# intuitive-robots/mdt_policy

Hardware: AMD Instinct MI355X
Metric: action-chunks/sec (10-step denoise, horizon=10) (higher is better)
Workload: dtype f32

## Files before the change

### include/mdt_hip_ops.h

```cpp
#ifndef MDT_HIP_OPS_H
#define MDT_HIP_OPS_H

#include <stdint.h>
#include "mdt_hip.h"

#ifdef __cplusplus
extern "C" {
#endif

enum { MDT_ACT_NONE = 0, MDT_ACT_GELU = 1, MDT_ACT_MISH = 2, MDT_ACT_SILU = 3,
       MDT_ACT_SWIGLU = 4  };
enum { MDT_HEAD_DENOISED = 0, MDT_HEAD_DDIM = 1, MDT_HEAD_RAW = 2,
       MDT_HEAD_PLAN = 3  };

int64_t mdt_op_packed_numel(int64_t N, int64_t K);

mdt_status mdt_op_pack_weight(const float *w, int64_t n_rows, int64_t K, float *packed, int64_t n_off,
                              int64_t N_total, void *stream);
mdt_status mdt_op_pack_weight_glu(const float *w, int64_t H2, int64_t K, float *packed, void *stream);

typedef struct {
    const float *A;
    int64_t lda;
    const float *Wp;
    const float *bias;
    float *out;
    int64_t ldo;
    int32_t M, N, K;
    int32_t ln;
    const float *ln_w, *ln_b;
    const float *mod;
    int64_t mod_stride;
    int32_t shift_off, scale_off;
    int32_t rows_per_sample;
    int32_t act;
    int32_t residual;
    int32_t gate_off;
    int32_t gin, gout, goff;
    const float *rowvec;
    int32_t batch;
    int64_t bs_a, bs_w, bs_out;
    const float *aux;
    int32_t aux_mode;
    int32_t a_parts;
    int64_t a_part_stride;
    float *a_merged;
    const void *Wp_split;
} mdt_gemm_args;

mdt_status mdt_op_gemm(const mdt_gemm_args *args, void *stream);

mdt_status mdt_op_mlp(const mdt_gemm_args *fc, const mdt_gemm_args *proj, float *parts, int64_t part_stride,
                      int32_t *n_parts, void *stream);
mdt_status mdt_op_pack_weight_split(const float *w, int64_t n_rows, int64_t K, void *image, void *stream);
mdt_status mdt_op_pack_weight_split_rows(const float *w, int64_t n_rows, int64_t K, void *image, int64_t n_off, void *stream);
mdt_status mdt_op_mlp_split(const mdt_gemm_args *fc, const mdt_gemm_args *proj, const void *fc_split, const void *proj_split,
                            float *parts, int64_t part_stride, int32_t *n_parts, void *stream);
void mdt_op_set_mlp_split(int32_t on);
void mdt_op_set_mlp_fuse_min(int32_t rows);
void mdt_op_set_side_jobs(int32_t on);
int64_t mdt_op_side_jobs_paired(void);
void mdt_op_trace_mlp(int32_t enable);
int32_t mdt_op_trace_mlp_read(float *us, int32_t cap);
int32_t mdt_op_trace_mlp_read_empty(float *us, int32_t cap);
mdt_status mdt_op_clock_stamp(uint64_t *out16, void *stream);
void mdt_op_set_ws_split(int32_t on);

void mdt_op_set_mlp_skew(int32_t v);

void mdt_op_set_gemm_geometry(int32_t geometry);

typedef struct {
    const float *q; int64_t ldq;
    const float *k; const float *v;
    int64_t ldkv;
    float *out; int64_t ldo;
    int32_t B, H, hd, Tq, Tk;
    int32_t causal;
    int32_t rope;
} mdt_attn_args;

mdt_status mdt_op_attention(const mdt_attn_args *args, void *stream);

mdt_status mdt_op_attn_proj(const mdt_gemm_args *proj, const float *qkv, int64_t ldq, int32_t hd, int32_t T, int32_t causal,
                            void *stream);
void mdt_op_set_attn_wide_min(int32_t rows);

mdt_status mdt_op_layernorm(const float *in, const float *w, const float *b, float *out, int64_t M, int32_t D,
                            void *stream);

typedef struct {
    const float *y;
    const float *ln_w;
    const float *ln_b;
    const float *Wp, *bp;
    const float *x;
    const float *sigma;
    int64_t sigma_stride;
    float *out;
    int32_t M, D, A, rows_per_sample;
    int32_t mode;
    const float *step;
    float sigma_data;
    float *y_next;
    const float *Wa, *ba;
    int32_t no_ln;
    int32_t y_parts;
    int64_t y_part_stride;
} mdt_head_args;

mdt_status mdt_op_head(const mdt_head_args *args, void *stream);

typedef struct {
    const float *kv; int64_t ldkv;
    const float *WqT_p;
    const float *bq;
    const float *Wo_p;
    float *U, *Wf;
    float *c;
    int32_t B, H, hd, D, Te;
} mdt_xfold_args;
mdt_status mdt_op_xattn_fold(const mdt_xfold_args *args, void *stream);

typedef struct {
    float *y;
    const float *ln_w, *ln_b;
    const float *U, *Wf, *c;
    const float *bo;
    int32_t B, H, D, Te, Ta;
    float *y_out;
} mdt_xapply_args;
mdt_status mdt_op_xattn_apply(const mdt_xapply_args *args, void *stream);

mdt_status mdt_op_xattn_gemm(const mdt_xapply_args *x, const mdt_gemm_args *g, void *stream);

mdt_status mdt_op_attn_xattn(const mdt_gemm_args *proj, const float *qkv, int64_t ldq, const mdt_xapply_args *x, int32_t hd,
                             int32_t T, void *stream);

mdt_status mdt_op_action_embed(const float *x, const float *sigma, int64_t sigma_stride, float sigma_data,
                               const float *WaT, const float *ba, float *y, int64_t M, int32_t A, int32_t D,
// ... 7 lines not shown
```

### mdt_policy_amd/_lib.py

```python
from __future__ import annotations

import ctypes as C
import os
import threading

from . import build as _build

c_float_p = C.POINTER(C.c_float)


class MDTHipError(RuntimeError):
    def __init__(self, status: int, message: str):
        super().__init__(f"libmdt_hip status {status}: {message}")
        self.status = status


class MDTConfig(C.Structure):
    _fields_ = [(n, C.c_int32) for n in (
        "arch", "embed_dim", "n_heads", "n_enc_layers", "n_dec_layers", "action_dim", "obs_dim", "goal_dim",
        "n_obs_token", "goal_seq_len", "action_seq_len", "use_mlp_goal", "use_modality_encoder", "use_abs_pos_emb",
        "use_rot_embed", "use_ada_conditioning", "use_noise_encoder", "linear_output", "bias")] + [
        ("sigma_data", C.c_float), ("no_goal_conditioning", C.c_int32), ("proprio_dim", C.c_int32),
        ("use_proprio", C.c_int32)]

# ... 119 lines not shown


class LinearBwdArgs(C.Structure):
    _fields_ = [("X", C.c_void_p), ("ldx", C.c_int64), ("dY", C.c_void_p), ("ldy", C.c_int64), ("Wt", C.c_void_p),
                ("dW", C.c_void_p), ("dbias", C.c_void_p), ("dX", C.c_void_p), ("ldxo", C.c_int64),
                ("accumulate_dw", C.c_int32), ("accumulate_dx", C.c_int32), ("M", C.c_int32), ("N", C.c_int32),
                ("K", C.c_int32), ("scratch", C.c_void_p), ("dx_act_u", C.c_void_p), ("dx_act", C.c_int32)]


class OptTensor(C.Structure):
    _fields_ = [("p", C.c_void_p), ("g", C.c_void_p), ("m", C.c_void_p), ("v", C.c_void_p), ("ema", C.c_void_p),
                ("numel", C.c_int64)]


class ResamplerConfig(C.Structure):
    _fields_ = [(n, C.c_int32) for n in ("dim", "depth", "dim_head", "heads", "num_latents", "num_time_embeds",
                                          "ff_mult", "activation")]


class MapPoolConfig(C.Structure):
    _fields_ = [(n, C.c_int32) for n in ("n_latents", "embed_dim", "output_dim", "n_heads", "mlp_hidden")]


class InfoNCEArgs(C.Structure):
    _fields_ = [("image_features", C.c_void_p), ("lang_features", C.c_void_p), ("logit_scale", C.c_void_p),
                ("batch", C.c_int32), ("dim", C.c_int32), ("mode", C.c_int32), ("loss", C.c_void_p),
                ("d_image", C.c_void_p), ("d_lang", C.c_void_p), ("d_logit_scale", C.c_void_p), ("scratch", C.c_void_p)]


INFONCE_MODE = {"symmetric": 0, "img_to_text": 1, "text_to_img": 2}
ARCH = {"mdtv": 0, "mdt": 1}
MODALITY = {"vis": 0, "lang": 1}
ACT = {"none": 0, "gelu": 1, "mish": 2, "silu": 3, "swiglu": 4}
HEAD = {"denoised": 0, "ddim": 1, "raw": 2}
RAW_OUTPUT, RAW_INPUT, SIGMA_SCALAR = 1, 2, 4

_VP, _I32, _I64, _F = C.c_void_p, C.c_int32, C.c_int64, C.c_float
SYMBOLS = [
    ("mdt_last_error", C.c_char_p, []),
    ("mdt_version", C.c_char_p, []),
    ("mdt_set_allocator", _I32, [_VP, _VP, _VP]),
    ("mdt_allocator_detach", _I32, []),
    ("mdt_create", _I32, [C.POINTER(MDTConfig), C.POINTER(_VP)]),
    ("mdt_destroy", _I32, [_VP]),
    ("mdt_param_count", _I64, [_VP]),
    ("mdt_param_name", C.c_char_p, [_VP, _I64]),
    ("mdt_param_numel", _I64, [_VP, _I64]),
    ("mdt_load_param", _I32, [_VP, C.c_char_p, _VP, _I64, _VP]),
    ("mdt_load_params", _I32, [_VP, _I32, C.POINTER(C.c_char_p), C.POINTER(C.c_void_p), C.POINTER(_I64), _VP]),
    ("mdt_reserve", _I32, [_VP, _I64]),
    ("mdt_ws_generation", _I64, [_VP]),
    ("mdt_encode", _I32, [_VP, _VP, _VP, _VP, _I32, _I32, _VP, _I64, _VP, _VP]),
    ("mdt_denoise_cached", _I32, [_VP, _VP, _VP, _I64, _I32, _VP, _VP]),
    ("mdt_forward", _I32, [_VP, _VP, _VP, _VP, _I32, _VP, _VP, _I64, _VP, _VP, _VP]),
    ("mdt_sample_ddim", _I32, [_VP, _VP, _VP, _VP, _I32, _VP, C.POINTER(C.c_float), _I32, _I64, _VP, _VP, _VP]),
    ("mdt_sample_ddim_dev", _I32, [_VP, _VP, _VP, _VP, _I32, _VP, _VP, _I32, _I64, _VP, _VP, _VP]),
    ("mdt_sample", _I32, [_VP, _VP, _VP, _VP, _I32, _VP, _I32, C.POINTER(SamplerParams), C.POINTER(C.c_float), _I32, _VP, _I32,
                          _I64, _VP, _VP, _VP]),
    ("mdt_sample_dev", _I32, [_VP, _VP, _VP, _VP, _I32, _VP, _I32, C.POINTER(SamplerParams), _VP, _I32, _VP, _I32, _I64, _VP,
                              _VP, _VP]),
    ("mdt_sampler_plan", _I32, [_I32, C.POINTER(SamplerParams), C.POINTER(C.c_float), _I32, C.POINTER(SamplerPlan)]),
    ("mdt_sample_dpm_adaptive", _I32, [_VP, _VP, _VP, _VP, _I32, _VP, C.c_float, C.c_float, C.POINTER(DpmAdaptiveParams), _I64,
                                       _VP, _VP, C.POINTER(DpmAdaptiveInfo), _VP]),
    ("mdt_dpm_control_init", _I32, [C.POINTER(DpmControl)] + [C.c_double] * 6),
    ("mdt_dpm_control_update", _I32, [C.POINTER(DpmControl), C.c_float, C.POINTER(C.c_int32)]),
    ("mdt_dpm_adaptive_plan", _I32, [_I32, C.c_float, C.c_float, C.POINTER(SamplerPlan)]),
    ("mdt_op_trace_mlp", None, [_I32]),
    ("mdt_op_trace_mlp_read", _I32, [_VP, _I32]),
    ("mdt_op_trace_mlp_read_empty", _I32, [_VP, _I32]),
    ("mdt_op_clock_stamp", _I32, [_VP, _VP]),
    ("mdt_op_set_ws_split", None, [_I32]),
    ("mdt_op_set_tn_split", None, [_I32]),
    ("mdt_loss_fwd", _I32, [_VP, _VP, _VP, _VP, _I32, _VP, _VP, _VP, _I64, _VP, _VP, _VP, _VP]),
    ("mdt_flops_per_chunk", C.c_double, [_VP, _I32]),
    ("mdt_fnv1_32", C.c_uint32, [C.c_char_p, C.c_uint64, C.c_uint32]),
    ("mdt_op_packed_numel", _I64, [_I64, _I64]),
    ("mdt_op_pack_weight", _I32, [_VP, _I64, _I64, _VP, _I64, _I64, _VP]),
    ("mdt_op_pack_weight_glu", _I32, [_VP, _I64, _I64, _VP, _VP]),
    ("mdt_op_gemm", _I32, [C.POINTER(GemmArgs), _VP]),
    ("mdt_op_mlp", _I32, [C.POINTER(GemmArgs), C.POINTER(GemmArgs), _VP, _I64, C.POINTER(_I32), _VP]),
    ("mdt_op_pack_weight_split", _I32, [_VP, _I64, _I64, _VP, _VP]),
    ("mdt_op_pack_weight_split_rows", _I32, [_VP, _I64, _I64, _VP, _I64, _VP]),
    ("mdt_op_mlp_split", _I32, [C.POINTER(GemmArgs), C.POINTER(GemmArgs), _VP, _VP, _VP, _I64, C.POINTER(_I32), _VP]),
    ("mdt_op_set_mlp_split", None, [_I32]),
    ("mdt_op_set_gemm_geometry", None, [_I32]),
    ("mdt_op_set_mlp_fuse_min", None, [_I32]),
    ("mdt_op_set_side_jobs", None, [_I32]),
    ("mdt_op_side_jobs_paired", _I64, []),
    ("mdt_op_set_mlp_skew", None, [_I32]),
    ("mdt_op_set_attn_wide_min", None, [_I32]),
    ("mdt_op_attention", _I32, [C.POINTER(AttnArgs), _VP]),
    ("mdt_op_attn_proj", _I32, [C.POINTER(GemmArgs), _VP, _I64, _I32, _I32, _I32, _VP]),
    ("mdt_op_xattn_fold", _I32, [C.POINTER(XFoldArgs), _VP]),
    ("mdt_op_xattn_apply", _I32, [C.POINTER(XApplyArgs), _VP]),
    ("mdt_op_attn_xattn", _I32, [C.POINTER(GemmArgs), _VP, _I64, C.POINTER(XApplyArgs), _I32, _I32, _VP]),
    ("mdt_op_xattn_gemm", _I32, [C.POINTER(XApplyArgs), C.POINTER(GemmArgs), _VP]),
    ("mdt_op_layernorm", _I32, [_VP, _VP, _VP, _VP, _I64, _I32, _VP]),
    ("mdt_op_head", _I32, [C.POINTER(HeadArgs), _VP]),
    ("mdt_op_action_embed", _I32, [_VP, _VP, _I64, _F, _VP, _VP, _VP, _I64, _I32, _I32, _I32, _VP]),
    ("mdt_train_prepare", _I32, [_VP]),
    ("mdt_grad_numel", _I64, [_VP]),
    ("mdt_grad_offset", _I64, [_VP, _I64]),
    ("mdt_train_loss_fwd", _I32, [_VP, _VP, _VP, _VP, _I32, _VP, _VP, _VP, _I64, C.POINTER(Dropout), _VP, _VP, _VP,
                                  C.POINTER(_I32), _VP]),
    ("mdt_train_loss_bwd", _I32, [_VP, _I32, _VP, _VP, _VP, _VP, _VP, _VP, _VP]),
    ("mdt_train_loss_bwd_stages", _I32, [_VP]),
    ("mdt_train_loss_bwd_stage", _I32, [_VP, _I32, _I32, _VP, _VP, _VP, _VP, _VP, _VP, _VP]),
    ("mdt_train_param_stage", _I32, [_VP, _I64]),
    ("mdt_train_encode_fwd", _I32, [_VP, _VP, _VP, _VP, _I32, _I32, _VP, _I64, C.POINTER(Dropout), _VP, C.POINTER(_I32),
                                    _VP]),
    ("mdt_train_encode_bwd", _I32, [_VP, _I32, _VP, _VP, _VP, _VP, _VP, _VP]),
    ("mdt_tape_release", _I32, [_VP, _I32]),
    ("mdt_denoise_vjp", _I32, [_VP, _VP, _VP, _VP, _I32, _VP, _VP, _VP, _I64, _VP, _VP, _VP]),
    ("mdt_op_pack_weight_t", _I32, [_VP, _I64, _I64, _I64, _VP, _I64, _I64, _VP]),
    ("mdt_op_pack_many", _I32, [_I32, C.POINTER(C.c_void_p), C.POINTER(_I32), C.POINTER(_I32), C.POINTER(C.c_void_p),
                                C.POINTER(C.c_void_p), _VP]),
    ("mdt_op_ln_fwd_train", _I32, [C.POINTER(LnTrainArgs), _VP]),
    ("mdt_op_ln_bwd", _I32, [C.POINTER(LnBwdArgs), _VP]),
    ("mdt_op_attn_bwd", _I32, [C.POINTER(AttnBwdArgs), _VP]),
    ("mdt_op_act_fwd", _I32, [_VP, _VP, _I64, _I32, _VP]),
    ("mdt_op_act_bwd", _I32, [_VP, _VP, _VP, _I64, _I32, _VP]),
    ("mdt_op_attn_fwd_train", _I32, [C.POINTER(AttnTrainArgs), _VP]),
    ("mdt_op_merge_fwd", _I32, [C.POINTER(MergeArgs), _VP]),
    ("mdt_op_merge_bwd", _I32, [C.POINTER(MergeArgs), _VP]),
    ("mdt_op_merge_ln_fwd", _I32, [C.POINTER(MergeArgs), C.POINTER(LnTrainArgs), _VP]),
    ("mdt_op_ln_bwd_merge", _I32, [C.POINTER(LnBwdArgs), C.POINTER(MergeArgs), _VP]),
    ("mdt_op_colsum", _I32, [_VP, _I64, _I64, _I64, _VP, _I32, _VP]),
    ("mdt_op_linear_bwd", _I32, [C.POINTER(LinearBwdArgs), _VP]),
    ("mdt_op_linear_bwd_scratch", _I64, [_I64, _I64, _I64]),
    ("mdt_op_linear_bwd_scratch_exact", _I64, [_I64, _I64, _I64]),
    ("mdt_op_multi_adamw", _I32, [C.POINTER(OptTensor), _I32, _F, _F, _F, _F, _F, _I64, _VP]),
    ("mdt_op_multi_ema", _I32, [C.POINTER(OptTensor), _I32, _F, _VP]),
    ("mdt_resampler_create", _I32, [C.POINTER(ResamplerConfig), C.POINTER(_VP)]),
    ("mdt_resampler_destroy", _I32, [_VP]),
    ("mdt_resampler_param_count", _I64, [_VP]),
    ("mdt_resampler_param_name", C.c_char_p, [_VP, _I64]),
    ("mdt_resampler_param_numel", _I64, [_VP, _I64]),
    ("mdt_resampler_load_param", _I32, [_VP, C.c_char_p, _VP, _I64, _VP]),
    ("mdt_resampler_forward", _I32, [_VP, _VP, _VP, _I64, _I32, _I32, _VP, _VP]),
    ("mdt_resampler_train_prepare", _I32, [_VP]),
    ("mdt_resampler_grad_numel", _I64, [_VP]),
    ("mdt_resampler_grad_offset", _I64, [_VP, _I64]),
    ("mdt_resampler_forward_train", _I32, [_VP, _VP, _VP, _I64, _I32, _I32, _VP, C.POINTER(_I32), _VP]),
    ("mdt_resampler_backward", _I32, [_VP, _I32, _VP, _VP, _VP, _VP]),
    ("mdt_resampler_tape_release", _I32, [_VP, _I32]),
    ("mdt_resampler_flops", C.c_double, [_VP, _I32, _I32]),
    ("mdt_map_pool_create", _I32, [C.POINTER(MapPoolConfig), C.POINTER(_VP)]),
    ("mdt_map_pool_destroy", _I32, [_VP]),
    ("mdt_map_pool_param_count", _I64, [_VP]),
    ("mdt_map_pool_param_name", C.c_char_p, [_VP, _I64]),
    ("mdt_map_pool_param_numel", _I64, [_VP, _I64]),
    ("mdt_map_pool_load_param", _I32, [_VP, C.c_char_p, _VP, _I64, _VP]),
    ("mdt_map_pool_forward", _I32, [_VP, _VP, _I64, _I32, _VP, _VP]),
    ("mdt_map_pool_train_prepare", _I32, [_VP]),
    ("mdt_map_pool_grad_numel", _I64, [_VP]),
    ("mdt_map_pool_grad_offset", _I64, [_VP, _I64]),
    ("mdt_map_pool_forward_train", _I32, [_VP, _VP, _I64, _I32, _VP, C.POINTER(_I32), _VP]),
    ("mdt_map_pool_backward", _I32, [_VP, _I32, _VP, _VP, _VP, _VP]),
    ("mdt_map_pool_tape_release", _I32, [_VP, _I32]),
    ("mdt_op_rms_fwd", _I32, [_VP, _VP, _VP, _I64, _I32, _F, _VP]),
    ("mdt_op_rms_bwd_scratch", _I64, [_I64, _I32]),
    ("mdt_op_rms_bwd", _I32, [_VP, _VP, _VP, _VP, _I32, _VP, _I32, _I64, _I32, _F, _VP, _VP]),
    ("mdt_op_rms_bwd_res", _I32, [_VP, _VP, _VP, _VP, _VP, _VP, _I32, _I64, _I32, _F, _VP, _VP]),
    ("mdt_op_scale_residual_fwd", _I32, [_VP, _VP, _VP, _VP, _I64, _I32, _VP]),
    ("mdt_op_scale_residual_bwd_scratch", _I64, [_I64, _I32]),
    ("mdt_op_scale_residual_bwd", _I32, [_VP, _VP, _VP, _VP, _VP, _I64, _I32, _VP, _VP]),
# ... 114 lines not shown
```

### mdt_policy_amd/csrc/mdt_internal.h

```cpp
#pragma once
#include <hip/hip_runtime.h>
#include <stdint.h>
#include <string.h>

#include "mdt_hip.h"
#include "mdt_hip_ops.h"
#include "mdt_resampler.h"
#include "mdt_hip_train.h"
#include "mdt_mae.h"

mdt_status mdt_fail(mdt_status st, const char* fmt, ...);

#define HIP_TRY(expr)                                                                                       \
    do {                                                                                                    \
        hipError_t _e = (expr);                                                                             \
        if (_e != hipSuccess) return mdt_fail(MDT_ERR_HIP, "%s failed: %s", #expr, hipGetErrorString(_e));  \
    } while (0)

#define MDT_TRY(expr)                      \
    do {                                   \
        mdt_status _s = (expr);            \
        if (_s != MDT_OK) return _s;       \
    } while (0)

#define LAUNCH(expr)                                                                                      \
    do {                                                                                                  \
        hipError_t _e = (expr);                                                                           \
        if (_e != hipSuccess) return mdt_fail(MDT_ERR_HIP, "%s: %s", #expr, hipGetErrorString(_e));       \
    } while (0)

struct Lin {
    float* wp = nullptr;
    float* bias = nullptr;
    int N = 0, K = 0;
    float* wt = nullptr;
    void* ws = nullptr;
};

struct Bump {
    float* base = nullptr;
    size_t off = 0;
    float* take(size_t n) {
        float* p = base ? base + off : nullptr;
        off += (n + 63) & ~(size_t)63;
        return p;
    }
};

static inline mdt_gemm_args gemm_args(const float* A, int64_t lda, const Lin& w, float* out, int64_t ldo, int M) {
    mdt_gemm_args g;
    memset(&g, 0, sizeof g);
    g.A = A; g.lda = lda; g.Wp = w.wp; g.Wp_split = w.ws; g.bias = w.bias; g.out = out; g.ldo = ldo;
    g.M = M; g.N = w.N; g.K = w.K;
    g.shift_off = -1; g.scale_off = -1; g.gate_off = -1; g.rows_per_sample = 1;
    g.gin = 1; g.gout = 1; g.goff = 0;
    return g;
}

hipError_t mdt_dev_malloc(void** p, size_t bytes);
hipError_t mdt_dev_free(void* p);

int mdt_gemm_kchunk(int K, int ln, int cap);
const float* mdt_zeros();
hipError_t mdt_launch_gemm(const mdt_gemm_args& a, hipStream_t s);
bool mdt_mlp_supported(const mdt_gemm_args& fc, const mdt_gemm_args& proj);
int mdt_mlp_slices(int D);
hipError_t mdt_launch_mlp(const mdt_gemm_args& fc, const mdt_gemm_args& proj, float* parts, int64_t part_stride, hipStream_t s);
bool mdt_mlp_split_supported(const mdt_gemm_args& fc, const mdt_gemm_args& proj);
bool mdt_mlp_split_enabled();
int mdt_split_min_rows();
hipError_t mdt_launch_mlp_split(const mdt_gemm_args& fc, const mdt_gemm_args& proj, const void* w1s, const void* w2s, float* parts,
                                int64_t part_stride, hipStream_t s);
hipError_t mdt_launch_pack_weight_split(const float* w, int n_rows, int K, void* image, hipStream_t s, int n_off = 0);
hipError_t mdt_launch_split_from_packed(const float* wp, int N, int K, void* image, hipStream_t s);
hipError_t mdt_launch_attention(const mdt_attn_args& a, const float* rope_cos, const float* rope_sin, hipStream_t s);
bool mdt_attn_proj_supported(const mdt_gemm_args& p, int H, int hd, int T, int rope);
hipError_t mdt_launch_attn_proj(const mdt_gemm_args& p, const float* qkv, int64_t ldq, int H, int hd, int T, int causal,
                                hipStream_t s);
bool mdt_attn_proj_wide_supported(const mdt_gemm_args& p, int H, int hd, int T, int causal, int rope);
hipError_t mdt_launch_attn_proj_wide(const mdt_gemm_args& p, const float* qkv, int64_t ldq, int H, int hd, int T, hipStream_t s);
bool mdt_attn_xattn_supported(const mdt_gemm_args& p, const mdt_xapply_args& x, int H, int hd, int T, int causal, int rope);
hipError_t mdt_launch_attn_xattn(const mdt_gemm_args& p, const float* qkv, int64_t ldq, const mdt_xapply_args& x, int H, int hd,
                                 int T, hipStream_t s);
hipError_t mdt_gemm_side_push(const mdt_gemm_args& a, hipStream_t s);
hipError_t mdt_gemm_side_push_front(const mdt_gemm_args& a, hipStream_t s);
hipError_t mdt_gemm_side_flush(hipStream_t s);
void mdt_gemm_side_drop();
size_t mdt_gemm_side_pending();
hipError_t mdt_gemm_side_launch_front(hipStream_t s);
hipError_t mdt_launch_layernorm(const float* in, const float* w, const float* b, float* out, int M, int D,
                                hipStream_t s, float* out2 = nullptr);
hipError_t mdt_launch_sigma_emb(const float* sigma, int64_t sstride, const float* freqs, float* out, int R, int D,
                                hipStream_t s);
constexpr int MDT_SCHED_MAX = 64;
struct mdt_sched_arg { float s[MDT_SCHED_MAX + 1]; };
hipError_t mdt_launch_sample_prep(const float* sigmas_dev, const float* sigmas_host, int n_steps, float* steps, const float* freqs,
                                  float* sig_e, int D, const float* x, float sd, const float* Wa, const float* ba, float* y, int M,
                                  int A, hipStream_t s);
hipError_t mdt_launch_sampler_prep(const float* sigmas_dev, const float* sigmas_host, int n_steps, int kind,
                                   const mdt_sampler_params& prm, mdt_sampler_plan_t* plan, const float* freqs, float* sig_e,
                                   int D, const float* x, const float* noise, int n_noise, float* y0, float* hist, float sd, const float* Wa,
                                   const float* ba, float* y, int M, int A, hipStream_t s);
hipError_t mdt_launch_sampler_first(const mdt_sampler_plan_t* plan, const float* x, const float* noise, int n_noise, float* y0,
                                    float* hist, float sd, const float* Wa, const float* ba, float* y, int M, int A, int D,
                                    hipStream_t s);
constexpr int MDT_DPM_PARTS = 256;
int mdt_dpm_error_parts(int64_t nel);
hipError_t mdt_launch_dpm_error(const float* lo, const float* hi, const float* prev, int64_t nel, float rtol, float atol,
                                float* part, hipStream_t s);
struct mdt_head_plan {
    const mdt_sampler_eval* e;
    const float* xs;
    float* hist;
    const float* noise;
    float* y_out;
    int64_t nel;
    int32_t n_noise;
};
hipError_t mdt_launch_head_plan(const mdt_head_args& a, const mdt_head_plan& pl, hipStream_t s);
hipError_t mdt_launch_action_embed(const float* x, const float* sigma, int64_t sstride, float sd, const float* Wa,
                                   const float* ba, float* y, int M, int A, int D, int rps, hipStream_t s);
hipError_t mdt_launch_head(const mdt_head_args& a, hipStream_t s);
hipError_t mdt_launch_noise_input(const float* act, const float* noise, const float* sigma, float* noised, int64_t n,
                                  int per_sample, hipStream_t s);
constexpr int MDT_LOSS_PARTS = 1024;
hipError_t mdt_launch_loss_reduce(const float* F, const float* act, const float* noised, const float* sigma, float sd,
                                  int64_t n, int per_sample, float* loss, float* part, hipStream_t s);
hipError_t mdt_launch_pack_weight(const float* w, int n_rows, int K, float* packed, int n_off, hipStream_t s);
hipError_t mdt_launch_pack_weight_glu(const float* w, int H, int K, float* packed, hipStream_t s);
enum { MDT_LOAD_RAW = 0, MDT_LOAD_PACK = 1, MDT_LOAD_PACK_T = 2, MDT_LOAD_TRANSPOSE = 3, MDT_LOAD_PAD_COLS = 4,
       MDT_LOAD_PACK_SPLIT = 5 };
struct mdt_load_entry {
    const float* src;
    float* dst;
    int32_t kind, rows, K;
    int32_t p0;
    int32_t p1;
    int32_t pad_;
};
hipError_t mdt_launch_multi_load(const mdt_load_entry* tab, const int2* blocks, int n_blocks, hipStream_t s);
hipError_t mdt_launch_transpose(const float* src, float* dst, int R, int Cc, hipStream_t s);
hipError_t mdt_launch_xattn_fold(const mdt_xfold_args& a, hipStream_t s);
hipError_t mdt_launch_xattn_fold_n(const mdt_xfold_args* sets, int n, hipStream_t s);
hipError_t mdt_launch_xattn_apply(const mdt_xapply_args& a, hipStream_t s);
bool mdt_xattn_gemm_supported(const mdt_xapply_args& x, const mdt_gemm_args& g);
hipError_t mdt_launch_xattn_gemm(const mdt_xapply_args& x, const mdt_gemm_args& g, hipStream_t s);
bool mdt_xattn_apply_supported(int D, int H, int Te, int Ta);
size_t mdt_xattn_lds_floats(int D, int H);
hipError_t mdt_launch_add_time_emb(const float* media, const float* tpe, const uint8_t* mask, float* out, int64_t B,
                                   int T, int n, int D, hipStream_t s);
hipError_t mdt_launch_bcast_rows(const float* src, float* out, int64_t B, int R, int D, hipStream_t s);
hipError_t mdt_launch_attention_long(const float* q, int64_t ldq, const float* k, const float* v, int64_t ldkv,
                                     float* out, int64_t ldo, int B, int H, int hd, int Tq, int Tk, float scale,
                                     hipStream_t s);
bool mdt_attention_long_supported(int hd, int Tq, int Tk);
// ... 77 lines not shown
```

### mdt_policy_amd/csrc/mdt_kernels.hip

```cpp
#include <hip/hip_runtime.h>

#include <atomic>
#include <stdint.h>
#include <stdlib.h>

#include <mutex>
#include <vector>

#include "mdt_internal.h"

#include "mdt_device.h"

#define MDT_TILES_TIMING_OWNER
#include "mdt_tiles.h"
#include "mdt_sampler_plan.h"
#include "mdt_tall.h"
#include "mdt_ws.h"
#include "mdt_mlp_split.h"

__global__ void k_pack_weight(const float* __restrict__ w, int n_rows, int K, float* __restrict__ packed,
                              int n_off, int K16) {
    const int64_t idx = (int64_t)blockIdx.x * blockDim.x + threadIdx.x;
    if (idx >= (int64_t)n_rows * K) return;
    const int n = (int)(idx / K), k = (int)(idx % K);
// ... 82 lines not shown
            const int nt = c >> 4, ni = c & 15, kc = k >> 4, h = (k & 15) >> 2;
            *(f32x4*)(e.dst + (((int64_t)nt * e.p1 + kc) * 64 + (ni + 16 * h)) * 4) = v;
            continue;
        }
        if (e.kind == MDT_LOAD_PACK_SPLIT) {
            const int K4 = e.K >> 2;
            if (idx >= (int64_t)e.rows * K4) continue;
            const int r = (int)(idx / K4), c = 4 * (int)(idx - (int64_t)r * K4);
            pack_split_quad(e.src, (char*)e.dst, r, c, e.K, e.p0);
            continue;
        }
        if (e.kind == MDT_LOAD_PACK) {
            const int K4 = e.K >> 2;
            if (idx >= (int64_t)e.rows * K4) continue;
            const int r = (int)(idx / K4), c = 4 * (int)(idx - (int64_t)r * K4);
            const int nn = r + e.p0;
            const int nt = nn >> 4, ni = nn & 15, kc = c >> 4, h = (c & 15) >> 2;
            *(f32x4*)(e.dst + (((int64_t)nt * (e.K >> 4) + kc) * 64 + (ni + 16 * h)) * 4) = *(const f32x4*)(e.src + (int64_t)r * e.K + c);
            continue;
        }
        if (idx >= n) continue;
        const float v = e.src[idx];
        if (e.kind == MDT_LOAD_RAW) {
            e.dst[idx] = v;
        } else {
            const int r = (int)(idx / e.K), c = (int)(idx - (int64_t)r * e.K);
            if (e.kind == MDT_LOAD_TRANSPOSE) {
                e.dst[(int64_t)c * e.rows + r] = v;
            } else {
                e.dst[(int64_t)r * e.p0 + c] = v;
            }
        }
    }
}
hipError_t mdt_launch_multi_load(const mdt_load_entry* tab, const int2* blocks, int n_blocks, hipStream_t s) {
    if (n_blocks < 1) return hipSuccess;
    hipLaunchKernelGGL(k_multi_load, dim3(n_blocks), dim3(256), 0, s, tab, blocks);
    return hipGetLastError();
}

#ifdef MDT_DEBUG_TIMING
extern "C" int mdt_debug_set_timing_buffer(unsigned long long* p) {
    return (int)hipMemcpyToSymbol(HIP_SYMBOL(g_dbg_ts), &p, sizeof(p));
}
#endif

template <int MTILES, int NTW, int NWAVES, int PRO, bool RES>
__global__ __launch_bounds__(64 * NWAVES) void k_gemm(mdt_gemm_args a, int kchunk, int grid_n,
                                                      const float* __restrict__ zeros) {
    extern __shared__ __attribute__((aligned(16))) float lds[];
    if (blockIdx.z) {
        a.A += (int64_t)blockIdx.z * a.bs_a; a.Wp += (int64_t)blockIdx.z * a.bs_w; a.out += (int64_t)blockIdx.z * a.bs_out;
    }
    const int logical = xcd_remap(blockIdx.x, gridDim.x);
    const int by = logical / grid_n, bx = logical - by * grid_n;
    gemm_tile<MTILES, NTW, NWAVES, PRO, RES, false>(a, kchunk, by, bx, lds, zeros, threadIdx.x);
}

template <int MTILES, int NTW, int NWAVES, int GLU>
__global__ __launch_bounds__(64 * NWAVES) void k_gemm_glu(mdt_gemm_args a, int kchunk, int grid_n, const float* __restrict__ zeros) {
    extern __shared__ __attribute__((aligned(16))) float lds[];
    const int logical = xcd_remap(blockIdx.x, gridDim.x);
    const int by = logical / grid_n, bx = logical - by * grid_n;
    gemm_tile<MTILES, NTW, NWAVES, PRO_PLAIN, false, false, 1, GLU>(a, kchunk, by, bx, lds, zeros, threadIdx.x);
}

template <int NTW, int PRO, int XP>
__global__ __launch_bounds__(512) void k_gemm_merge(mdt_gemm_args a, int kchunk, int grid_n, const float* __restrict__ zeros) {
    extern __shared__ __attribute__((aligned(16))) float lds[];
    const int logical = xcd_remap(blockIdx.x, gridDim.x);
    const int by = logical / grid_n, bx = logical - by * grid_n;
    gemm_tile<2, NTW, 8, PRO, false, false, XP>(a, kchunk, by, bx, lds, zeros, threadIdx.x);
}

template <int NTW2, int PRO>
__global__ __launch_bounds__(512) void k_mlp(mdt_gemm_args f, mdt_gemm_args p, float* __restrict__ parts, int64_t part_stride,
                                             int n_slices, const float* __restrict__ zeros, int skew) {
    extern __shared__ __attribute__((aligned(16))) float lds[];
    const int logical = xcd_remap(blockIdx.x, gridDim.x);
    const int by = logical / n_slices, s = logical - by * n_slices;
    mlp_tile<NTW2, PRO>(f, p, parts, part_stride, by, s, lds, zeros, threadIdx.x, skew);
}

template <int NTW2, int PRO>
__global__ __launch_bounds__(512) void k_mlp_split(mdt_gemm_args f, mdt_gemm_args p, const char* __restrict__ w1s, const char* __restrict__ w2s,
                                                   float* __restrict__ parts, int64_t part_stride, int n_slices, int gm,
                                                   const float* __restrict__ zeros) {
    extern __shared__ __attribute__((aligned(16))) char lds_c[];
    const int total = gm * n_slices, per = (total + 7) >> 3;
    const int i = blockIdx.x >> 3, w = (blockIdx.x & 7) * per + i;
    if (i >= per || w >= total) return;
    const int s = w / gm, by = w - s * gm;
    mlp_split_tile<NTW2, PRO>(f, p, w1s, w2s, parts, part_stride, by, s, lds_c, zeros, threadIdx.x);
}

template <int MTILES, int NTW, int NWAVES, int LW, bool RES>
__global__ __launch_bounds__(64 * (NWAVES + LW)) void k_gemm_pipe(mdt_gemm_args a, int kchunk, int grid_n,
                                                                 const float* __restrict__ zeros) {
    extern __shared__ __attribute__((aligned(16))) float lds[];
    constexpr int MT = MTILES * 16;
    constexpr bool KSTEP_PRIO = true;
    constexpr int R = NTW == 1 ? 6 : (NTW == 2 ? 4 : 3);
    const f32x4 zero4 = (f32x4){0.f, 0.f, 0.f, 0.f};
    const int tid = threadIdx.x, lane = tid & 63, wave = tid >> 6;
    const bool loader = wave >= NWAVES;
    if (blockIdx.z) {
        a.A += (int64_t)blockIdx.z * a.bs_a; a.Wp += (int64_t)blockIdx.z * a.bs_w; a.out += (int64_t)blockIdx.z * a.bs_out;
    }
    const int logical = xcd_remap(blockIdx.x, gridDim.x);
    const int by = logical / grid_n, bx = logical - by * grid_n;
    const int m0 = by * MT;
    const int N16 = a.N >> 4, K16 = a.K >> 4;
    const int nt0 = (bx * NWAVES + min(wave, NWAVES - 1)) * NTW;
    const bool active = !loader && nt0 < N16;
    const int stride = kchunk + 4;
    const int bufsz = MT * stride;
    const int nchunks = (a.K + kchunk - 1) / kchunk;

    auto stage = [&](int c) {
        constexpr int RG = 2 * LW, U = MT / RG;
        const int lt = tid - 64 * NWAVES, rg = lt >> 5, l32 = lt & 31;
        const int k0 = c * kchunk, n4 = min(kchunk, a.K - k0) >> 2;
        float* dst = lds + (c & 1) * bufsz;
        f32x4 st[U][3];
#pragma unroll
        for (int u = 0; u < U; ++u) {
            const int64_t m = min(m0 + rg + RG * u, a.M - 1);
#pragma unroll
            for (int v = 0; v < 3; ++v) st[u][v] = ldg4(a.A + m * a.lda + k0 + 4 * min(l32 + 32 * v, n4 - 1));
        }
#pragma unroll
        for (int u = 0; u < U; ++u) {
            const int row = rg + RG * u;
#pragma unroll
            for (int v = 0; v < 3; ++v)
                if (l32 + 32 * v < n4) *(f32x4*)(dst + row * stride + 4 * (l32 + 32 * v)) = sel4(m0 + row < a.M, st[u][v], zero4);
        }
    };

    WStream wp[NTW];
    f32x4 ring[R][NTW];
    f32x4 acc[MTILES][NTW];
    const int nq = 4 * (lane >> 4);
    const bool gated = RES && a.gate_off >= 0;
    int ncol[NTW];
    constexpr int NRES = RES ? NTW : 1;
    f32x4 bias_v[NTW], gate_v[MTILES][NRES], res_v[MTILES][NRES];
    float* optr[MTILES];
    if (loader) {
        stage(0);
    } else {
#pragma unroll
        for (int j = 0; j < NTW; ++j) {
            const int nt = min(nt0 + j, N16 - 1);
            wp[j] = wstream(a.Wp, (int64_t)nt * K16 * 256 + lane * 4);
        }
#pragma unroll
        for (int u = 0; u < R - 1; ++u)
#pragma unroll
            for (int j = 0; j < NTW; ++j) ring[u][j] = wld4(wp[j] + min(u, K16 - 1) * 256);
#pragma unroll
        for (int i = 0; i < MTILES; ++i)
#pragma unroll
            for (int j = 0; j < NTW; ++j) acc[i][j] = zero4;
        const float* biasp = a.bias != nullptr ? a.bias : zeros;
        const float* rvp = a.rowvec != nullptr ? a.rowvec : zeros;
#pragma unroll
        for (int j = 0; j < NTW; ++j) {
            ncol[j] = min(nt0 + j, N16 - 1) * 16 + nq;
            bias_v[j] = ldg4(biasp + ncol[j]) + ldg4(rvp + ncol[j]);
        }
#pragma unroll
        for (int i = 0; i < MTILES; ++i) {
            const int m = min(m0 + i * 16 + (lane & 15), a.M - 1);
            const int64_t orow =
                a.gin == 1 ? (int64_t)m * a.gout + a.goff : (int64_t)(m / a.gin) * a.gout + (m % a.gin) + a.goff;
// ... 318 lines not shown
__global__ __launch_bounds__(512) void k_gemm_smallm2(mdt_gemm_args a, mdt_gemm_args b, int nxa, int nya, const float* __restrict__ zeros) {
    __shared__ float s_stat[32];
    __shared__ __attribute__((aligned(16))) float red[8 * 64 * 4];
    const int na = nxa * nya;
    if ((int)blockIdx.x < na) gemm_smallm_tile<false>(a, blockIdx.x % nxa, (blockIdx.x / nxa) * 16, s_stat, red, zeros, threadIdx.x);
    else {
        const int i = blockIdx.x - na, nxb = b.N >> 4;
        gemm_smallm_tile<false>(b, i % nxb, (i / nxb) * 16, s_stat, red, zeros, threadIdx.x);
    }
}

static constexpr int GEMM_MID_MAX = 1400;
template <int NPP>
__global__ __launch_bounds__(512) void k_xattn_gemm_smallm(mdt_xapply_args x, mdt_gemm_args a, const float* __restrict__ zeros) {
    extern __shared__ __attribute__((aligned(16))) float lds[];
    __shared__ float s_stat[32];
    __shared__ __attribute__((aligned(16))) float red[8 * 64 * 4];
    const int b = blockIdx.y, ys = x.D + 4;
    float* yo = lds;
    xattn_tile<NPP, false, false, 512, 0, true>(x, b, lds + 16 * ys, zeros, threadIdx.x, nullptr, 0, nullptr, yo, ys, blockIdx.x == 0);
    __syncthreads();
    gemm_smallm_tile<false, true>(a, blockIdx.x, b * x.Ta, s_stat, red, zeros, threadIdx.x, yo, ys, x.Ta);
}

static constexpr int GEMM_SMALLM_MAX = 15, GEMM_SMALLM_ROWS = 512;

int mdt_gemm_kchunk(int K, int ln, int cap) {
    if (ln || K <= 512) return K;
    for (int c = cap; c >= 16; c -= 16)
        if (K % c == 0) return c;
    return 16;
}

template <int MTILES, int NTW, int NWAVES>
static hipError_t launch_gemm_pro(const mdt_gemm_args& a, int kchunk, hipStream_t s) {
    if (!a.ln) return launch_gemm_t<MTILES, NTW, NWAVES, PRO_PLAIN>(a, kchunk, s);
    if (a.mod != nullptr && a.shift_off >= 0)
        return a.mod_stride == 0 ? launch_gemm_t<MTILES, NTW, NWAVES, PRO_LN_MOD_BCAST>(a, kchunk, s)
                                 : launch_gemm_t<MTILES, NTW, NWAVES, PRO_LN_MOD_ROWS>(a, kchunk, s);
    return launch_gemm_t<MTILES, NTW, NWAVES, PRO_LN>(a, kchunk, s);
}

int g_mdt_gemm_force = 0;

static bool w_image_ok(int64_t N, int64_t K) { return N * K < ((int64_t)1 << 30); }

bool mdt_attn_proj_supported(const mdt_gemm_args& p, int H, int hd, int T, int rope) {
    return w_image_ok(p.N, p.K) && H == 8 && (hd == 16 || hd == 32 || hd == 48 || hd == 64) && p.K == H * hd && T >= 1 && T <= 16 && p.M >= T &&
           p.M % T == 0 && p.M / T <= 64 && (p.rows_per_sample == T || p.M == T) && !rope &&
           !(p.N & 15) && p.gin == 1 && p.gout == 1 && p.goff == 0 && !p.ln && p.act == MDT_ACT_NONE && p.rowvec == nullptr &&
           p.batch <= 1;
}

template <int HD>
static hipError_t launch_attn_proj_t(const mdt_gemm_args& p, const float* qkv, int64_t ldq, int T, int causal, hipStream_t s) {
    const size_t lds = (size_t)8 * 3 * T * (HD + 4) * sizeof(float);
    static size_t lds_attr_dev[MAX_DEVICES] = {0};
    size_t& lds_attr = lds_attr_dev[current_device()];
    if (lds > 48 * 1024 && lds > lds_attr) {
        hipError_t e = hipFuncSetAttribute((const void*)k_attn_proj_smallm<HD>, hipFuncAttributeMaxDynamicSharedMemorySize, (int)lds);
        if (e != hipSuccess) return e;
        lds_attr = lds;
    }
    hipLaunchKernelGGL((k_attn_proj_smallm<HD>), dim3(p.N >> 4, p.M / T), dim3(512), lds, s, p, qkv, ldq, T, causal,
                       1.0f / sqrtf((float)HD), g_zeros);
    return hipGetLastError();
}

hipError_t mdt_launch_attn_proj(const mdt_gemm_args& p, const float* qkv, int64_t ldq, int H, int hd, int T, int causal,
                                hipStream_t s) {
    if (!mdt_attn_proj_supported(p, H, hd, T, 0)) return hipErrorInvalidValue;
    hipError_t ze = ensure_zeros();
    if (ze != hipSuccess) return ze;
    switch (hd) {
        case 16: return launch_attn_proj_t<16>(p, qkv, ldq, T, causal, s);
        case 32: return launch_attn_proj_t<32>(p, qkv, ldq, T, causal, s);
        case 48: return launch_attn_proj_t<48>(p, qkv, ldq, T, causal, s);
        default: return launch_attn_proj_t<64>(p, qkv, ldq, T, causal, s);
    }
}

static hipError_t launch_gemm_merge(const mdt_gemm_args& a, hipStream_t s);
static bool gemm_ln_split_applies(const mdt_gemm_args& a);
static hipError_t launch_gemm_ln_split(const mdt_gemm_args& a, hipStream_t s);

bool mdt_attn_proj_wide_supported(const mdt_gemm_args& p, int H, int hd, int T, int causal, int rope) {
    return w_image_ok(p.N, p.K) && H == 8 && (hd == 16 || hd == 32 || hd == 48) && p.K == H * hd && T >= 1 && T <= 16 && causal && !rope && p.residual &&
           p.M >= T && p.M % T == 0 && p.rows_per_sample == T && !(p.N & 15) && p.gin == 1 && p.gout == 1 && p.goff == 0 && !p.ln &&
           p.act == MDT_ACT_NONE && p.rowvec == nullptr && p.batch <= 1 && !p.aux_mode;
}

template <int HD, int TKC>
static hipError_t launch_attn_proj_wide_t(const mdt_gemm_args& p, const mdt_attn_pro& ap, hipStream_t s) {
    const int gn = (p.N + 127) / 128, gm = (p.M + 31) / 32;
    const size_t lds = ((size_t)32 * (p.K + 4) + (size_t)(32 + 2 * 48) * (4 * HD + 16)) * sizeof(float);
    static size_t lds_attr_dev[MAX_DEVICES] = {0};
    size_t& lds_attr = lds_attr_dev[current_device()];
    if (lds > lds_attr) {
        hipError_t e = hipFuncSetAttribute((const void*)k_attn_proj_wide<HD, TKC>, hipFuncAttributeMaxDynamicSharedMemorySize, (int)lds);
        if (e != hipSuccess) return e;
        lds_attr = lds;
    }
    hipLaunchKernelGGL((k_attn_proj_wide<HD, TKC>), dim3(gn * gm), dim3(512), lds, s, p, ap, gn, g_zeros);
    return hipGetLastError();
}

hipError_t mdt_launch_attn_proj_wide(const mdt_gemm_args& p, const float* qkv, int64_t ldq, int H, int hd, int T, hipStream_t s) {
    if (!mdt_attn_proj_wide_supported(p, H, hd, T, 1, 0)) return hipErrorInvalidValue;
    hipError_t ze = ensure_zeros();
    if (ze != hipSuccess) return ze;
    mdt_attn_pro ap;
    ap.qkv = qkv; ap.ldq = ldq; ap.T = T; ap.scale = 1.0f / sqrtf((float)hd);
    const bool t10 = T <= 10;
    switch (hd) {
        case 16: return t10 ? launch_attn_proj_wide_t<16, 10>(p, ap, s) : launch_attn_proj_wide_t<16, 16>(p, ap, s);
        case 32: return t10 ? launch_attn_proj_wide_t<32, 10>(p, ap, s) : launch_attn_proj_wide_t<32, 16>(p, ap, s);
        default: return t10 ? launch_attn_proj_wide_t<48, 10>(p, ap, s) : launch_attn_proj_wide_t<48, 16>(p, ap, s);
    }
}

bool mdt_xattn_apply_supported(int D, int H, int Te, int Ta);

bool mdt_attn_xattn_supported(const mdt_gemm_args& p, const mdt_xapply_args& x, int H, int hd, int T, int causal, int rope) {
    return mdt_attn_proj_wide_supported(p, H, hd, T, causal, rope) && hd == 48 && p.N == p.K && p.ldo == p.N && x.y == p.out &&
           x.D == p.N && x.H == H && H == 8 && x.Ta == T && (int64_t)x.B * T == p.M &&
           mdt_xattn_apply_supported(x.D, x.H, x.Te, x.Ta);
}

template <int HD, int TKC>
static hipError_t launch_attn_xattn_t(const mdt_gemm_args& p, const mdt_attn_pro& at, const mdt_xapply_args& x, hipStream_t s) {
    const int D = 8 * HD;
    const size_t lds = ((size_t)16 * (D + 4) + (size_t)48 * (D + 16)) * sizeof(float);
    static bool attr_dev[MAX_DEVICES] = {false};
    bool& attr = attr_dev[current_device()];
    if (!attr) {
        hipError_t e = hipFuncSetAttribute((const void*)k_attn_xattn<HD, TKC>, hipFuncAttributeMaxDynamicSharedMemorySize, (int)lds);
        if (e != hipSuccess) return e;
        attr = true;
    }
    hipLaunchKernelGGL((k_attn_xattn<HD, TKC>), dim3(x.B), dim3(512), lds, s, p, at, x, g_zeros);
    return hipGetLastError();
}

hipError_t mdt_launch_attn_xattn(const mdt_gemm_args& p, const float* qkv, int64_t ldq, const mdt_xapply_args& x, int H, int hd,
                                 int T, hipStream_t s) {
    if (!mdt_attn_xattn_supported(p, x, H, hd, T, 1, 0) || ldq != 3 * (int64_t)p.K) return hipErrorInvalidValue;
    hipError_t ze = ensure_zeros();
    if (ze != hipSuccess) return ze;
    mdt_attn_pro at;
    at.qkv = qkv; at.ldq = ldq; at.T = T; at.scale = 1.0f / sqrtf((float)hd);
    return T <= 10 ? launch_attn_xattn_t<48, 10>(p, at, x, s) : launch_attn_xattn_t<48, 16>(p, at, x, s);
}

static thread_local std::vector<mdt_gemm_args> g_side_jobs;
static thread_local size_t g_side_next = 0;
static bool smallm_shape_ok(const mdt_gemm_args& a) {
    return a.M >= 1 && a.M <= 15 && (!a.ln || a.K <= 512) && a.batch <= 1 && a.K <= 4096 && !a.aux_mode && a.a_parts <= 1 &&
           a.N <= ZEROS_FLOATS && a.K <= ZEROS_FLOATS && !(a.N & 15) && (int64_t)a.N * a.K < ((int64_t)1 << 30);
}
static std::atomic<int> g_side_override{-1};
static std::atomic<int64_t> g_side_paired{0};
static bool side_enabled() {
    return g_side_override.load(std::memory_order_relaxed) != 0 && g_mdt_gemm_force == 0;
}
extern "C" void mdt_op_set_side_jobs(int32_t on) { g_side_override.store(on < 0 ? -1 : (on != 0)); }
extern "C" int64_t mdt_op_side_jobs_paired(void) { return g_side_paired.load(); }
hipError_t mdt_gemm_side_push(const mdt_gemm_args& a, hipStream_t s) {
// ... 87 lines not shown
    if (a.M >= 8192 && a.N % 64 == 0 && (a.N > 384 || a.K > 384) && a.batch <= 1 && mdt_gemm_tall_supported(a)) geo = 23;
    if (a.batch > 1) geo = 5;
    if (g_mdt_gemm_force > 0) geo = g_mdt_gemm_force;
    if (geo == 30) {
        if (mdt_gemm_ws_supported(a)) return launch_gemm_ws(a, s);
        geo = 0;
    }
    if (geo >= 10 && (geo != 23 || !mdt_gemm_tall_supported(a))) geo = 0;
    switch (geo) {
        case 23: return launch_gemm_tall<2, 2, 2, 3, 1>(a, s);
        case 1: return launch_gemm_pro<2, 1, 4>(a, mdt_gemm_kchunk(a.K, a.ln, 384), s);
        case 2:
            if (!a.ln && a.K > 512) {
                const int kc = mdt_gemm_kchunk(a.K, 0, 384);
                return a.residual ? launch_gemm_pipe_r<2, 1, 8, 4, true>(a, kc, s)
                                  : launch_gemm_pipe_r<2, 1, 8, 4, false>(a, kc, s);
            }
            return launch_gemm_pro<2, 1, 8>(a, mdt_gemm_kchunk(a.K, a.ln, 768), s);
        case 3: return launch_gemm_pro<2, 3, 8>(a, mdt_gemm_kchunk(a.K, a.ln, 768), s);
        case 4: return launch_gemm_pro<2, 4, 8>(a, mdt_gemm_kchunk(a.K, a.ln, 768), s);
        case 6: {
            if (!a.ln && a.K > 512 && !a.aux_mode && (int64_t)((a.M + 15) / 16) * ((a.N + 63) / 64) <= 256) {
                const int kc = mdt_gemm_kchunk(a.K, 0, 384);
                return a.residual ? launch_gemm_pipe_r<1, 1, 4, 2, true>(a, kc, s) : launch_gemm_pipe_r<1, 1, 4, 2, false>(a, kc, s);
            }
            return launch_gemm_pro<1, 1, 4>(a, mdt_gemm_kchunk(a.K, a.ln, 384), s);
        }
        case 7: return launch_gemm_pro<4, 2, 4>(a, mdt_gemm_kchunk(a.K, a.ln, 384), s);
        case 8: return launch_gemm_pro<2, 4, 4>(a, mdt_gemm_kchunk(a.K, a.ln, 384), s);
        case 9: return launch_gemm_pro<2, 3, 4>(a, mdt_gemm_kchunk(a.K, a.ln, 384), s);
        default: return launch_gemm_pro<2, 2, 4>(a, mdt_gemm_kchunk(a.K, a.ln, 384), s);
    }
}

extern "C" void mdt_op_set_gemm_geometry(int32_t geo) { g_mdt_gemm_force = geo; }

bool mdt_mlp_supported(const mdt_gemm_args& f, const mdt_gemm_args& p) {
    const int D = f.K;
    return D >= 128 && D <= 512 && D % 128 == 0 && f.N == 4 * D && p.N == D && p.K == 4 * D && f.ln && f.batch <= 1 &&
           f.gin == 1 && f.gout == 1 && f.goff == 0 && f.rowvec == nullptr && !f.aux_mode && f.a_parts <= 1 && f.M >= 1 &&
           f.rows_per_sample >= 1 && p.rows_per_sample >= 1;
}
int mdt_mlp_slices(int D) { return 4 * D / 512; }

static int g_mlp_skew = -1;
static int mlp_skew() { return g_mlp_skew < 0 ? 18 | 256 : g_mlp_skew; }
extern "C" void mdt_op_set_mlp_skew(int32_t v) { g_mlp_skew = v < 0 ? -1 : (v & 0x1ff); }

template <int NTW2, int PRO>
static hipError_t launch_mlp_t(const mdt_gemm_args& f, const mdt_gemm_args& p, float* parts, int64_t part_stride, hipStream_t s) {
    const int S = mdt_mlp_slices(f.K), gm = (f.M + 31) / 32;
    const size_t lds = (size_t)32 * (f.K + 4 + 516) * sizeof(float) + 16 * sizeof(int);
    const int skew = mlp_skew();
    static size_t lds_attr_dev[MAX_DEVICES] = {0};
    size_t& lds_attr = lds_attr_dev[current_device()];
    if (lds > lds_attr) {
        hipError_t e = hipFuncSetAttribute((const void*)k_mlp<NTW2, PRO>, hipFuncAttributeMaxDynamicSharedMemorySize, (int)lds);
        if (e != hipSuccess) return e;
        lds_attr = lds;
    }
    hipLaunchKernelGGL((k_mlp<NTW2, PRO>), dim3(gm * S), dim3(512), lds, s, f, p, parts, part_stride, S, g_zeros, skew);
    return hipGetLastError();
}
template <int NTW2>
static hipError_t launch_mlp_pro(const mdt_gemm_args& f, const mdt_gemm_args& p, float* parts, int64_t part_stride, hipStream_t s) {
    if (f.mod != nullptr && f.shift_off >= 0)
        return f.mod_stride == 0 ? launch_mlp_t<NTW2, PRO_LN_MOD_BCAST>(f, p, parts, part_stride, s)
                                 : launch_mlp_t<NTW2, PRO_LN_MOD_ROWS>(f, p, parts, part_stride, s);
    return launch_mlp_t<NTW2, PRO_LN>(f, p, parts, part_stride, s);
}
hipError_t mdt_launch_mlp(const mdt_gemm_args& f, const mdt_gemm_args& p, float* parts, int64_t part_stride, hipStream_t s) {
    if (!mdt_mlp_supported(f, p)) return hipErrorInvalidValue;
    hipError_t ze = ensure_zeros();
    if (ze != hipSuccess) return ze;
    switch (f.K / 128) {
        case 1: return launch_mlp_pro<1>(f, p, parts, part_stride, s);
        case 2: return launch_mlp_pro<2>(f, p, parts, part_stride, s);
        case 3: return launch_mlp_pro<3>(f, p, parts, part_stride, s);
        default: return launch_mlp_pro<4>(f, p, parts, part_stride, s);
    }
}

template <int ND, int NTW, int PRO, int XP>
__global__ __launch_bounds__(512) void k_gemm_ln_split(mdt_gemm_args a, int grid_n, const float* __restrict__ zeros) {
    extern __shared__ __attribute__((aligned(16))) char lds_c[];
    const int logical = xcd_remap(blockIdx.x, gridDim.x);
    const int by = logical / grid_n, bx = logical - by * grid_n;
    gemm_ln_split_tile<ND, NTW, PRO, XP>(a, by, bx, lds_c, zeros, threadIdx.x);
}
template <int ND, int NTW, int PRO, int XP>
static hipError_t launch_gemm_ln_split_t(const mdt_gemm_args& a, hipStream_t s) {
    const int gn = a.N / (8 * NTW * 16), gm = (a.M + 31) / 32;
    const int lds = 3 * 32 * (2 * 128 * ND + 32);
    static bool attr_dev[MAX_DEVICES] = {false};
    bool& done = attr_dev[current_device()];
    if (!done) {
        hipError_t e = hipFuncSetAttribute((const void*)k_gemm_ln_split<ND, NTW, PRO, XP>, hipFuncAttributeMaxDynamicSharedMemorySize, lds);
        if (e != hipSuccess) return e;
        done = true;
    }
    hipLaunchKernelGGL((k_gemm_ln_split<ND, NTW, PRO, XP>), dim3(gn * gm), dim3(512), lds, s, a, gn, g_zeros);
    return hipGetLastError();
}
template <int ND, int NTW, int PRO>
static hipError_t launch_gemm_ln_split_x(const mdt_gemm_args& a, hipStream_t s) {
    switch (a.a_parts) {
        case 2: return launch_gemm_ln_split_t<ND, NTW, PRO, 2>(a, s);
        case 3: return launch_gemm_ln_split_t<ND, NTW, PRO, 3>(a, s);
        case 4: return launch_gemm_ln_split_t<ND, NTW, PRO, 4>(a, s);
        default: return launch_gemm_ln_split_t<ND, NTW, PRO, 1>(a, s);
    }
}
template <int ND, int NTW>
static hipError_t launch_gemm_ln_split_pro(const mdt_gemm_args& a, hipStream_t s) {
    if (a.mod != nullptr && a.shift_off >= 0)
        return a.mod_stride == 0 ? launch_gemm_ln_split_x<ND, NTW, PRO_LN_MOD_BCAST>(a, s) : launch_gemm_ln_split_x<ND, NTW, PRO_LN_MOD_ROWS>(a, s);
    return launch_gemm_ln_split_x<ND, NTW, PRO_LN>(a, s);
}
static bool gemm_ln_split_applies(const mdt_gemm_args& a) {
    return a.Wp_split != nullptr && mdt_mlp_split_enabled() && a.ln && (a.K == 384 || a.K == 512) && a.N % 384 == 0 &&
           a.M >= mdt_split_min_rows() && a.batch <= 1 && !a.residual && a.gin == 1 && a.gout == 1 && a.goff == 0 && a.rowvec == nullptr && !a.aux_mode &&
           a.a_parts <= 4 && (a.lda & 3) == 0 && (a.ldo & 3) == 0 && g_mdt_gemm_force == 0;
}
static hipError_t launch_gemm_ln_split(const mdt_gemm_args& a, hipStream_t s) {
    return a.K == 512 ? launch_gemm_ln_split_pro<4, 3>(a, s) : launch_gemm_ln_split_pro<3, 3>(a, s);
}

static int g_mlp_split = -1;
bool mdt_mlp_split_enabled() {
    if (g_mlp_split < 0) { const char* e = getenv("MDT_HIP_MLP_SPLIT"); g_mlp_split = e ? atoi(e) : 1; }
    return g_mlp_split != 0;
}
extern "C" void mdt_op_set_mlp_split(int32_t on) { g_mlp_split = on < 0 ? -1 : (on != 0); }
int mdt_split_min_rows() { return 768; }
bool mdt_mlp_split_supported(const mdt_gemm_args& f, const mdt_gemm_args& p) {
    return mdt_mlp_supported(f, p);
}
template <int NTW2, int PRO>
static hipError_t launch_mlp_split_t(const mdt_gemm_args& f, const mdt_gemm_args& p, const void* w1s, const void* w2s, float* parts,
                                     int64_t part_stride, hipStream_t s) {
    const int S = mdt_mlp_slices(f.K), gm = (f.M + 31) / 32;
    const int lds = mlp_split_lds_bytes(128 * NTW2);
    static bool attr_dev[MAX_DEVICES] = {false};
    bool& done = attr_dev[current_device()];
    if (!done) {
        hipError_t e = hipFuncSetAttribute((const void*)k_mlp_split<NTW2, PRO>, hipFuncAttributeMaxDynamicSharedMemorySize, lds);
        if (e != hipSuccess) return e;
        done = true;
    }
    const int per = (gm * S + 7) / 8;
    hipLaunchKernelGGL((k_mlp_split<NTW2, PRO>), dim3(8 * per), dim3(512), lds, s, f, p, (const char*)w1s, (const char*)w2s, parts,
                       part_stride, S, gm, g_zeros);
    return hipGetLastError();
}
template <int NTW2>
static hipError_t launch_mlp_split_pro(const mdt_gemm_args& f, const mdt_gemm_args& p, const void* w1s, const void* w2s, float* parts,
                                       int64_t part_stride, hipStream_t s) {
    if (f.mod != nullptr && f.shift_off >= 0)
        return f.mod_stride == 0 ? launch_mlp_split_t<NTW2, PRO_LN_MOD_BCAST>(f, p, w1s, w2s, parts, part_stride, s)
                                 : launch_mlp_split_t<NTW2, PRO_LN_MOD_ROWS>(f, p, w1s, w2s, parts, part_stride, s);
    return launch_mlp_split_t<NTW2, PRO_LN>(f, p, w1s, w2s, parts, part_stride, s);
}
hipError_t mdt_launch_mlp_split(const mdt_gemm_args& f, const mdt_gemm_args& p, const void* w1s, const void* w2s, float* parts,
                                int64_t part_stride, hipStream_t s) {
    if (!mdt_mlp_split_supported(f, p) || !w1s || !w2s) return hipErrorInvalidValue;
    hipError_t ze = ensure_zeros();
    if (ze != hipSuccess) return ze;
    switch (f.K / 128) {
        case 1: return launch_mlp_split_pro<1>(f, p, w1s, w2s, parts, part_stride, s);
        case 2: return launch_mlp_split_pro<2>(f, p, w1s, w2s, parts, part_stride, s);
        case 3: return launch_mlp_split_pro<3>(f, p, w1s, w2s, parts, part_stride, s);
        default: return launch_mlp_split_pro<4>(f, p, w1s, w2s, parts, part_stride, s);
    }
}

template <int NTW, int PRO, int XP>
static hipError_t launch_gemm_merge_t(const mdt_gemm_args& a, hipStream_t s) {
    const int NTC = 8 * NTW * 16;
    const int gn = (a.N + NTC - 1) / NTC, gm = (a.M + 31) / 32;
    const size_t lds = (size_t)32 * (a.K + 4) * sizeof(float);
    static size_t lds_attr_dev[MAX_DEVICES] = {0};
    size_t& lds_attr = lds_attr_dev[current_device()];
    if (lds > lds_attr) {
        hipError_t e = hipFuncSetAttribute((const void*)k_gemm_merge<NTW, PRO, XP>, hipFuncAttributeMaxDynamicSharedMemorySize, (int)lds);
        if (e != hipSuccess) return e;
        lds_attr = lds;
    }
    hipLaunchKernelGGL((k_gemm_merge<NTW, PRO, XP>), dim3(gn * gm), dim3(512), lds, s, a, a.K, gn, g_zeros);
    return hipGetLastError();
}
template <int NTW, int PRO>
static hipError_t launch_gemm_merge_x(const mdt_gemm_args& a, hipStream_t s) {
    switch (a.a_parts) {
        case 2: return launch_gemm_merge_t<NTW, PRO, 2>(a, s);
        case 3: return launch_gemm_merge_t<NTW, PRO, 3>(a, s);
        case 4: return launch_gemm_merge_t<NTW, PRO, 4>(a, s);
        default: return hipErrorInvalidValue;
    }
}
template <int NTW>
static hipError_t launch_gemm_merge_pro(const mdt_gemm_args& a, hipStream_t s) {
    if (a.mod != nullptr && a.shift_off >= 0)
        return a.mod_stride == 0 ? launch_gemm_merge_x<NTW, PRO_LN_MOD_BCAST>(a, s) : launch_gemm_merge_x<NTW, PRO_LN_MOD_ROWS>(a, s);
    return launch_gemm_merge_x<NTW, PRO_LN>(a, s);
}
static hipError_t launch_gemm_merge(const mdt_gemm_args& a, hipStream_t s) {
    if (!a.ln || a.K > 512 || a.residual || a.batch > 1 || a.aux_mode || a.a_parts > 4 || (a.N & 15)) return hipErrorInvalidValue;
    return (a.N % 384 == 0) ? launch_gemm_merge_pro<3>(a, s) : launch_gemm_merge_pro<4>(a, s);
}

template <int HD, int TKC, bool ROPE>
__global__ __launch_bounds__(256) void k_attn(mdt_attn_args a, const float* __restrict__ rope_cos,
                                              const float* __restrict__ rope_sin, float scale) {
    extern __shared__ __attribute__((aligned(16))) float lds[];
    const int b = xcd_remap(blockIdx.x, gridDim.x);
    attn_tile<HD, TKC, ROPE, false>(a, rope_cos, rope_sin, scale, b, blockIdx.y, gridDim.y, lds, threadIdx.x);
}

template <int HD, int TKC, bool ROPE>
static hipError_t launch_attn_tt(const mdt_attn_args& a, const float* rc, const float* rs, hipStream_t s) {
    constexpr int LP = HD == 48 ? 3 : (HD >= 32 ? 2 : 1);
    const int hs = (a.H % 2 == 0 && a.B >= 64) ? 2 : 1;
    const int Hl = a.H / hs;
    const size_t lds = ((size_t)(a.Tq + 2 * a.Tk) * Hl * HD + (size_t)Hl * a.Tq * 16 * LP) * sizeof(float);
    static size_t lds_attr_dev[MAX_DEVICES] = {0};
    size_t& lds_attr = lds_attr_dev[current_device()];
    if (lds > lds_attr) {
        hipError_t e = hipFuncSetAttribute((const void*)k_attn<HD, TKC, ROPE>, hipFuncAttributeMaxDynamicSharedMemorySize,
                                           (int)lds);
        if (e != hipSuccess) return e;
        lds_attr = lds;
    }
    hipLaunchKernelGGL((k_attn<HD, TKC, ROPE>), dim3(a.B, hs), dim3(256), lds, s, a, rc, rs, 1.0f / sqrtf((float)HD));
    return hipGetLastError();
}

template <int HD>
static hipError_t launch_attn_t(const mdt_attn_args& a, const float* rc, const float* rs, hipStream_t s) {
    if constexpr (HD >= 32) {
        if (a.rope) {
            if (a.Tk <= 4) return launch_attn_tt<HD, 4, true>(a, rc, rs, s);
            if (a.Tk <= 10) return launch_attn_tt<HD, 10, true>(a, rc, rs, s);
            return launch_attn_tt<HD, 16, true>(a, rc, rs, s);
        }
    }
    if (a.Tk <= 4) return launch_attn_tt<HD, 4, false>(a, rc, rs, s);
    if (a.Tk <= 10) return launch_attn_tt<HD, 10, false>(a, rc, rs, s);
    return launch_attn_tt<HD, 16, false>(a, rc, rs, s);
}

// ... 740 lines not shown
```

### mdt_policy_amd/csrc/mdt_mlp_split.h

```cpp
#pragma once
#include <hip/hip_runtime.h>
#include <stdint.h>

#include "mdt_device.h"
#include "mdt_internal.h"
#include "mdt_tiles.h"
#include "mdt_ws.h"

template <int NT, int R>
struct SplitRing {
    mdt_bf16x8 w[R][NT][3];
    __amdgpu_buffer_rsrc_t rs;
    unsigned voff[NT];
    __device__ __forceinline__ void open(const void* image, int64_t first_byte, int64_t tile_stride, int lane) {
        rs = __builtin_amdgcn_make_buffer_rsrc((void*)image, 0, 0xffffffffu, 0x00020000);
#pragma unroll
        for (int j = 0; j < NT; ++j) voff[j] = (unsigned)(first_byte + j * tile_stride) + 16u * (unsigned)lane;
    }
    __device__ __forceinline__ void request(int slot, int kk) {
#pragma unroll
        for (int j = 0; j < NT; ++j)
#pragma unroll
            for (int p = 0; p < 3; ++p)
                w[slot][j][p] = __builtin_bit_cast(mdt_bf16x8, __builtin_amdgcn_raw_buffer_load_b128(rs, voff[j], (kk * 3 + p) * 1024, 0));
    }
};

template <int NT, int K32, int R>
__device__ __forceinline__ void split_phase(SplitRing<NT, R>& ring, const char* xa, int rowb, int part, int lane, f32x4 (&acc)[2][NT]) {
    const int aoff = (lane & 15) * rowb + (lane >> 4) * 16;
    mdt_bf16x8 x1[2], x2[2], x3[2];
#pragma unroll
    for (int i = 0; i < 2; ++i) {
        const char* q = xa + aoff + i * 16 * rowb;
        x1[i] = *(const mdt_bf16x8*)q; x2[i] = *(const mdt_bf16x8*)(q + part); x3[i] = *(const mdt_bf16x8*)(q + 2 * part);
    }
#pragma unroll
    for (int kk = 0; kk < K32; ++kk) {
        const int u = kk % R, un = (kk + R - 1) % R;
        const bool nx = kk + 1 < K32;
        if (kk + R - 1 < K32) ring.request(un, kk + R - 1);
        const char* p0 = xa + aoff + (kk + 1) * 64;
        const char* p1 = p0 + 16 * rowb;
        MDT_SCHED_PIN
#pragma unroll
        for (int j = 0; j < NT; ++j) {
            acc[0][j] = __builtin_amdgcn_mfma_f32_16x16x32_bf16(ring.w[u][j][0], x3[0], acc[0][j], 0, 0, 0);
            acc[1][j] = __builtin_amdgcn_mfma_f32_16x16x32_bf16(ring.w[u][j][0], x3[1], acc[1][j], 0, 0, 0);
        }
        MDT_SCHED_PIN
        if (nx) { x3[0] = *(const mdt_bf16x8*)(p0 + 2 * part); x3[1] = *(const mdt_bf16x8*)(p1 + 2 * part); }
        MDT_SCHED_PIN
#pragma unroll
        for (int j = 0; j < NT; ++j) {
            acc[0][j] = __builtin_amdgcn_mfma_f32_16x16x32_bf16(ring.w[u][j][1], x2[0], acc[0][j], 0, 0, 0);
            acc[1][j] = __builtin_amdgcn_mfma_f32_16x16x32_bf16(ring.w[u][j][1], x2[1], acc[1][j], 0, 0, 0);
        }
#pragma unroll
        for (int j = 0; j < NT; ++j) {
            acc[0][j] = __builtin_amdgcn_mfma_f32_16x16x32_bf16(ring.w[u][j][0], x2[0], acc[0][j], 0, 0, 0);
            acc[1][j] = __builtin_amdgcn_mfma_f32_16x16x32_bf16(ring.w[u][j][0], x2[1], acc[1][j], 0, 0, 0);
        }
        MDT_SCHED_PIN
        if (nx) { x2[0] = *(const mdt_bf16x8*)(p0 + part); x2[1] = *(const mdt_bf16x8*)(p1 + part); }
        MDT_SCHED_PIN
#pragma unroll
        for (int j = 0; j < NT; ++j) {
            acc[0][j] = __builtin_amdgcn_mfma_f32_16x16x32_bf16(ring.w[u][j][2], x1[0], acc[0][j], 0, 0, 0);
            acc[1][j] = __builtin_amdgcn_mfma_f32_16x16x32_bf16(ring.w[u][j][2], x1[1], acc[1][j], 0, 0, 0);
        }
#pragma unroll
        for (int j = 0; j < NT; ++j) {
            acc[0][j] = __builtin_amdgcn_mfma_f32_16x16x32_bf16(ring.w[u][j][1], x1[0], acc[0][j], 0, 0, 0);
            acc[1][j] = __builtin_amdgcn_mfma_f32_16x16x32_bf16(ring.w[u][j][1], x1[1], acc[1][j], 0, 0, 0);
        }
#pragma unroll
        for (int j = 0; j < NT; ++j) {
            acc[0][j] = __builtin_amdgcn_mfma_f32_16x16x32_bf16(ring.w[u][j][0], x1[0], acc[0][j], 0, 0, 0);
            acc[1][j] = __builtin_amdgcn_mfma_f32_16x16x32_bf16(ring.w[u][j][0], x1[1], acc[1][j], 0, 0, 0);
        }
        MDT_SCHED_PIN
        if (nx) { x1[0] = *(const mdt_bf16x8*)p0; x1[1] = *(const mdt_bf16x8*)p1; }
        MDT_SCHED_PIN
    }
}

__host__ __device__ constexpr int mlp_split_lds_bytes(int D) {
    const int xs = 3 * 32 * (2 * D + 32), hs = 3 * 32 * (2 * 512 + 32);
    return xs > hs ? xs : hs;
}

template <int NTW2, int PRO>
__device__ __forceinline__ void mlp_split_tile(const mdt_gemm_args& f, const mdt_gemm_args& p, const char* __restrict__ w1s,
                                               const char* __restrict__ w2s, float* __restrict__ parts, int64_t part_stride, int by,
                                               int s, char* lds, const float* __restrict__ zeros, int tid) {
    constexpr int MTILES = 2, NWAVES = 8, MT = 32, HS = 512, NTW1 = 4, R = 2;
    constexpr int D = 128 * NTW2, K32a = D / 32, K32b = HS / 32;
    constexpr int ROWB1 = 2 * D + 32, PART1 = MT * ROWB1, ROWB2 = 2 * HS + 32, PART2 = MT * ROWB2;
    static_assert(NTW2 >= 1 && NTW2 <= 4, "D <= 512");
    const f32x4 zero4 = (f32x4){0.f, 0.f, 0.f, 0.f};
    const int lane = tid & 63, wave = tid >> 6;
    const int m0 = by * MT;
    const int nq = 4 * (lane >> 4);
    char* xs = lds;
    char* hs = lds;

    const int nt1 = (s * NWAVES + wave) * NTW1;
    SplitRing<NTW1, R> ring1;
    ring1.open(w1s, (int64_t)nt1 * K32a * 3072, (int64_t)K32a * 3072, lane);
#pragma unroll
    for (int u = 0; u < R - 1; ++u) ring1.request(u, u);
    f32x4 b1[NTW1];
    {
        const float* bp = f.bias != nullptr ? f.bias : zeros;
#pragma unroll
        for (int j = 0; j < NTW1; ++j) b1[j] = ldg4(bp + (nt1 + j) * 16 + nq);
    }
    gemm_stage_tile<MTILES, NWAVES, PRO, false, 1, 2, true>(f, (float*)xs, ROWB1, m0, 0, D, zeros, tid, lane, wave);
    __syncthreads();
    f32x4 acc1[MTILES][NTW1];
#pragma unroll
    for (int i = 0; i < MTILES; ++i)
#pragma unroll
        for (int j = 0; j < NTW1; ++j) acc1[i][j] = zero4;
    split_phase<NTW1, K32a, R>(ring1, xs, ROWB1, PART1, lane, acc1);

    const int K32p = p.K >> 5;
    SplitRing<NTW2, R> ring2;
    ring2.open(w2s, ((int64_t)(wave * NTW2) * K32p + (int64_t)s * K32b) * 3072, (int64_t)K32p * 3072, lane);
#pragma unroll
    for (int u = 0; u < R - 1; ++u) ring2.request(u, u);
    constexpr bool EARLY = NTW2 <= 3;
    f32x4 acc2[MTILES][NTW2], b2[NTW2], gate_v[MTILES][NTW2], res_v[MTILES][NTW2];
    int ncol[NTW2];
#pragma unroll
    for (int j = 0; j < NTW2; ++j) ncol[j] = (wave * NTW2 + j) * 16 + nq;
    const bool gated = p.mod != nullptr && p.gate_off >= 0;
    auto load_gate_res = [&]() __attribute__((always_inline)) {
#pragma unroll
        for (int i = 0; i < MTILES; ++i) {
            const int64_t m = min(m0 + i * 16 + (lane & 15), f.M - 1);
            const float* gp = gated ? p.mod + p.gate_off + (p.mod_stride == 0 ? 0 : (m / p.rows_per_sample) * p.mod_stride)
                                    : zeros;
            const float* rp = s == 0 ? f.A + m * f.lda : zeros;
#pragma unroll
            for (int j = 0; j < NTW2; ++j) {
                gate_v[i][j] = ldg4(gp + ncol[j]);
                res_v[i][j] = ldg4(rp + ncol[j]);
            }
        }
    };
    {
        const float* bp = (s == 0 && p.bias != nullptr) ? p.bias : zeros;
#pragma unroll
        for (int j = 0; j < NTW2; ++j) b2[j] = ldg4(bp + ncol[j]);
#pragma unroll
        for (int i = 0; i < MTILES; ++i)
#pragma unroll
            for (int j = 0; j < NTW2; ++j) acc2[i][j] = zero4;
        if constexpr (EARLY) load_gate_res();
    }
    __syncthreads();
#pragma unroll
    for (int i = 0; i < MTILES; ++i)
#pragma unroll
        for (int j = 0; j < NTW1; ++j) {
            mdt_bf16x4 p1, p2, p3;
            split3_bf16(apply_act(acc1[i][j] + b1[j], f.act), p1, p2, p3);
            char* q = hs + split_slot(i * 16 + (lane & 15), (wave * NTW1 + j) * 16 + nq, ROWB2);
            *(mdt_bf16x4*)q = p1;
            *(mdt_bf16x4*)(q + PART2) = p2;
            *(mdt_bf16x4*)(q + 2 * PART2) = p3;
        }
    __syncthreads();
    split_phase<NTW2, K32b, R>(ring2, hs, ROWB2, PART2, lane, acc2);

    if constexpr (!EARLY) load_gate_res();
    float* out = parts + (int64_t)s * part_stride;
#pragma unroll
    for (int i = 0; i < MTILES; ++i) {
        const int m = m0 + i * 16 + (lane & 15);
#pragma unroll
        for (int j = 0; j < NTW2; ++j) {
            f32x4 v = acc2[i][j] + b2[j];
            v = res_v[i][j] + (gated ? gate_v[i][j] * v : v);
            if (m < f.M) st4(out + (int64_t)m * p.ldo + ncol[j], v);
        }
    }
}

template <int ND, int NTW, int PRO, int XP>
__device__ __forceinline__ void gemm_ln_split_tile(const mdt_gemm_args& a, int by, int bx, char* lds, const float* __restrict__ zeros, int tid) {
    constexpr int MTILES = 2, NWAVES = 8, MT = 32, R = 2;
    constexpr int D = 128 * ND, K32 = D / 32, ROWB = 2 * D + 32, PART = MT * ROWB;
    static_assert(ND >= 1 && ND <= 4, "D <= 512");
    const f32x4 zero4 = (f32x4){0.f, 0.f, 0.f, 0.f};
    const int lane = tid & 63, wave = tid >> 6;
    const int m0 = by * MT, nq = 4 * (lane >> 4);
    char* xs = lds;
    const int nt0 = (bx * NWAVES + wave) * NTW;
    SplitRing<NTW, R> ring;
    ring.open(a.Wp_split, (int64_t)nt0 * K32 * 3072, (int64_t)K32 * 3072, lane);
#pragma unroll
    for (int u = 0; u < R - 1; ++u) ring.request(u, u);
    f32x4 bias_v[NTW];
    {
        const float* bp = a.bias != nullptr ? a.bias : zeros;
#pragma unroll
        for (int j = 0; j < NTW; ++j) bias_v[j] = ldg4(bp + (nt0 + j) * 16 + nq);
    }
    gemm_stage_tile<MTILES, NWAVES, PRO, false, XP, (NTW <= 3 && XP <= 3) ? 1 : 2, true>(a, (float*)xs, ROWB, m0, 0, D, zeros, tid, lane, wave,
                                                                                         bx == 0 ? a.a_merged : nullptr);
    __syncthreads();
    f32x4 acc[MTILES][NTW];
#pragma unroll
    for (int i = 0; i < MTILES; ++i)
#pragma unroll
        for (int j = 0; j < NTW; ++j) acc[i][j] = zero4;
    split_phase<NTW, K32, R>(ring, xs, ROWB, PART, lane, acc);
#pragma unroll
    for (int i = 0; i < MTILES; ++i) {
        const int m = m0 + i * 16 + (lane & 15);
#pragma unroll
        for (int j = 0; j < NTW; ++j)
            if (m < a.M) st4(a.out + (int64_t)m * a.ldo + (nt0 + j) * 16 + nq, apply_act(acc[i][j] + bias_v[j], a.act));
    }
}
```

### mdt_policy_amd/csrc/mdt_model.hip

```cpp
#include <hip/hip_runtime.h>

#include <algorithm>
#include <cmath>
#include <cstdarg>
#include <cstdio>
#include <cstdlib>
#include <cstring>
#include <string>
#include <unordered_map>
#include <vector>

#include "mdt_internal.h"
#include "mdt_sampler_plan.h"

static thread_local std::string g_err;

mdt_status mdt_fail(mdt_status st, const char* fmt, ...) {
    char buf[1024];
    va_list ap;
    va_start(ap, fmt);
    vsnprintf(buf, sizeof buf, fmt, ap);
    va_end(ap);
    g_err = buf;
    return st;
// ... 119 lines not shown
            p.lin = &l; p.w_slot = (int)m->slots.size() - 1; p.b_slot = bias ? p.w_slot + 1 : -1; p.rows = rows; p.n_off = n_off;
            m->parts.push_back(p);
        }
        if (bias) add_slot(prefix + ".bias", rows, SLOT_RAW, l.bias ? l.bias + n_off : nullptr, 0, 0, 0);
    };
    auto raw = [&](float*& p, const std::string& name, int64_t n) {
        p = b.take(n);
        add_slot(name, n, SLOT_RAW, p, 0, 0, 0);
    };
    auto add_extra = [&](const std::string& name, int64_t numel, int kind, float* dst, int rows, int K, int n_off = 0) {
        if (!fill_slots) return;
        Slot s;
        s.name = name; s.numel = numel; s.kind = kind; s.dst = dst; s.rows = rows; s.K = K; s.n_off = n_off;
        m->extra.push_back(s);
    };
    const std::string P = "inner_model.";
    const bool xb = c.bias != 0;

    if (c.arch == MDT_ARCH_MDT && c.use_abs_pos_emb)
        raw(m->pos_emb, P + "pos_emb", (int64_t)(c.goal_seq_len + c.action_seq_len) * D);
    lin_begin(m->tok, D, O, true);
    lin_part(m->tok, P + "tok_emb", D, 0, true);
    if (c.arch == MDT_ARCH_MDT) {
        lin_begin(m->incam, D, O, true);
        lin_part(m->incam, P + "incam_embed", D, 0, true);
    }
    auto goal_mlp = [&](Lin& l0, Lin& l2, const std::string& nm) {
        if (c.use_mlp_goal) {
            lin_begin(l0, 2 * D, G, true);
            lin_part(l0, P + nm + ".0", 2 * D, 0, true);
            lin_begin(l2, D, 2 * D, true);
            lin_part(l2, P + nm + ".2", D, 0, true);
        } else {
            lin_begin(l2, D, G, true);
            lin_part(l2, P + nm, D, 0, true);
        }
    };
    goal_mlp(m->goal0, m->goal2, "goal_emb");
    if (c.use_modality_encoder) goal_mlp(m->lang0, m->lang2, "lang_emb");

    auto attn_qkv = [&](Lin& qkv, const std::string& pre) {
        lin_begin(qkv, 3 * D, D, true);
        lin_part(qkv, pre + ".key", D, D, true);
        lin_part(qkv, pre + ".query", D, 0, true);
        lin_part(qkv, pre + ".value", D, 2 * D, true);
        if (D % 128 == 0 && D <= 512) {
            qkv.ws = b.take((size_t)3 * D * D * 6 / 4);
            add_extra(pre + ".key.weight", (int64_t)D * D, SLOT_PACK_SPLIT, (float*)qkv.ws, D, D, D);
            add_extra(pre + ".query.weight", (int64_t)D * D, SLOT_PACK_SPLIT, (float*)qkv.ws, D, D, 0);
            add_extra(pre + ".value.weight", (int64_t)D * D, SLOT_PACK_SPLIT, (float*)qkv.ws, D, D, 2 * D);
        }
    };
    auto block_common_a = [&](EncBlock& e, const std::string& pre) {
        raw(e.ln1_w, pre + ".ln_1.weight", D);
        if (xb) raw(e.ln1_b, pre + ".ln_1.bias", D);
        attn_qkv(e.qkv, pre + ".attn");
        lin_begin(e.proj, D, D, xb);
        lin_part(e.proj, pre + ".attn.c_proj", D, 0, xb);
    };
    auto block_common_b = [&](EncBlock& e, const std::string& pre) {
        raw(e.ln2_w, pre + ".ln_2.weight", D);
        if (xb) raw(e.ln2_b, pre + ".ln_2.bias", D);
        lin_begin(e.fc, 4 * D, D, xb);
        lin_part(e.fc, pre + ".mlp.c_fc", 4 * D, 0, xb);
        lin_begin(e.proj2, D, 4 * D, xb);
        lin_part(e.proj2, pre + ".mlp.c_proj", D, 0, xb);
        if (D % 128 == 0 && D <= 512) {
            e.fc.ws = b.take((size_t)4 * D * D * 6 / 4);
            e.proj2.ws = b.take((size_t)4 * D * D * 6 / 4);
            add_extra(pre + ".mlp.c_fc.weight", (int64_t)4 * D * D, SLOT_PACK_SPLIT, (float*)e.fc.ws, 4 * D, D);
            add_extra(pre + ".mlp.c_proj.weight", (int64_t)4 * D * D, SLOT_PACK_SPLIT, (float*)e.proj2.ws, D, 4 * D);
        }
    };
    if (!fill_slots) { m->enc.assign(m->Le, EncBlock()); m->dec.assign(m->Ld, DecBlock()); }
    for (int l = 0; l < m->Le; ++l) {
        const std::string pre = P + "encoder.blocks." + std::to_string(l);
        block_common_a(m->enc[l], pre);
        block_common_b(m->enc[l], pre);
    }
    raw(m->enc_ln_w, P + "encoder.ln.weight", D);
    if (xb) raw(m->enc_ln_b, P + "encoder.ln.bias", D);

    lin_begin(m->kv_all, m->Ld * 2 * D, D, true);
    if (m->cond == COND_ADALN) lin_begin(m->mod_all, m->Ld * 6 * D, D, true);
    for (int l = 0; l < m->Ld; ++l) {
        const std::string pre = P + "decoder.blocks." + std::to_string(l);
        DecBlock& d = m->dec[l];
        block_common_a(d, pre);
        lin_part(m->kv_all, pre + ".cross_att.key", D, l * 2 * D, true);
        lin_begin(d.xq, D, D, true);
        lin_part(d.xq, pre + ".cross_att.query", D, 0, true);
        d.xq_pT = b.take((size_t)D * D);
        add_extra(pre + ".cross_att.query.weight", (int64_t)D * D, SLOT_PACK_T, d.xq_pT, D, D);
        lin_part(m->kv_all, pre + ".cross_att.value", D, l * 2 * D + D, true);
        lin_begin(d.xproj, D, D, xb);
        lin_part(d.xproj, pre + ".cross_att.c_proj", D, 0, xb);
        raw(d.ln3_w, pre + ".ln3.weight", D);
        raw(d.ln3_b, pre + ".ln3.bias", D);
        block_common_b(d, pre);
        if (m->cond == COND_ADALN) lin_part(m->mod_all, pre + ".adaLN_zero.modulation.1", 6 * D, l * 6 * D, true);
    }
    raw(m->dec_ln_w, P + "decoder.ln.weight", D);
    if (xb) raw(m->dec_ln_b, P + "decoder.ln.bias", D);
    if (c.use_proprio) {
        m->prop0_T = b.take((size_t)2 * D * c.proprio_dim);
        add_slot(P + "proprio_emb.0.weight", (int64_t)2 * D * c.proprio_dim, SLOT_TRANSPOSE, m->prop0_T, 2 * D, c.proprio_dim, 0);
        raw(m->prop0_b, P + "proprio_emb.0.bias", 2 * D);
        lin_begin(m->prop2, D, 2 * D, true);
        lin_part(m->prop2, P + "proprio_emb.2", D, 0, true);
    }
    lin_begin(m->sig1, 2 * D, D, true);
    lin_part(m->sig1, P + "sigma_emb.1", 2 * D, 0, true);
    lin_begin(m->sig3, D, 2 * D, true);
    lin_part(m->sig3, P + "sigma_emb.3", D, 0, true);
    m->Wa = b.take((size_t)D * A);
    add_slot(P + "action_emb.weight", (int64_t)D * A, SLOT_TRANSPOSE, m->Wa, D, A, 0);
    raw(m->ba, P + "action_emb.bias", D);
    if (c.linear_output) {
        raw(m->Wp, P + "action_pred.weight", (int64_t)A * D);
        raw(m->bp, P + "action_pred.bias", A);
    } else {
        m->HH = c.arch == MDT_ARCH_MDTV ? 100 : D;
        m->HP = (m->HH + 15) / 16 * 16;
        lin_begin(m->head0, m->HP, D, true);
        lin_part(m->head0, P + "action_pred.0", m->HH, 0, true);
        m->Wp = b.take((size_t)A * m->HP);
        add_slot(P + "action_pred.2.weight", (int64_t)A * m->HH, SLOT_PAD_COLS, m->Wp, A, m->HH, m->HP);
        raw(m->bp, P + "action_pred.2.bias", A);
    }
    m->freqs = b.take(D / 2);
    m->rope_cos = b.take(16 * 16);
    m->rope_sin = b.take(16 * 16);
}

static bool is_ignored_param(const mdt_model* m, const std::string& name) {
    auto ends_with = [&](const char* suf) {
        const size_t n = strlen(suf);
        return name.size() >= n && name.compare(name.size() - n, n, suf) == 0;
    };
    if (!m->cfg.use_proprio && name.rfind("inner_model.proprio_emb.", 0) == 0) return true;
    if (ends_with(".rotary_pos_emb.freqs")) return true;
    if (name == "inner_model.pos_emb") return true;
    if (!m->cfg.use_modality_encoder && name.rfind("inner_model.lang_emb", 0) == 0) return false;
    return false;
}

extern "C" mdt_status mdt_create(const mdt_config* cfg, mdt_model** out) {
    if (!cfg || !out) return fail(MDT_ERR_INVALID_ARG, "mdt_create: null argument");
    const mdt_config& c = *cfg;
    if (c.arch != MDT_ARCH_MDTV && c.arch != MDT_ARCH_MDT) return fail(MDT_ERR_INVALID_ARG, "unknown arch %d", c.arch);
    if (c.goal_seq_len != 1) return fail(MDT_ERR_UNSUPPORTED, "goal_seq_len must be 1");
    if (c.embed_dim <= 0 || c.embed_dim % 16 || c.embed_dim > 512)
        return fail(MDT_ERR_UNSUPPORTED, "embed_dim %d: need a multiple of 16, <= 512", c.embed_dim);
    if (c.n_heads <= 0 || c.embed_dim % c.n_heads) return fail(MDT_ERR_INVALID_ARG, "embed_dim %% n_heads != 0");
    const int hd = c.embed_dim / c.n_heads;
    if (hd != 16 && hd != 32 && hd != 48 && hd != 64)
        return fail(MDT_ERR_UNSUPPORTED, "head dim %d: supported 16/32/48/64", hd);
    if (c.use_rot_embed && hd < 32)
        return fail(MDT_ERR_INVALID_ARG, "use_rot_embed needs head dim >= 32 (rotary dim is 32; the reference asserts)");
    if (c.obs_dim % 16 || c.goal_dim % 16 || c.obs_dim <= 0 || c.goal_dim <= 0)
        return fail(MDT_ERR_UNSUPPORTED, "obs_dim / goal_dim must be positive multiples of 16");
    if (c.goal_dim == 2 * c.obs_dim)
        return fail(MDT_ERR_UNSUPPORTED, "goal_dim == 2*obs_dim triggers the reference's goal truncation "
                                         "(mdtv_transformer.py:252-253); not implemented");
    if (c.action_dim < 1 || c.action_dim > 16) return fail(MDT_ERR_UNSUPPORTED, "action_dim must be 1..16");
    if (c.action_seq_len < 1 || c.action_seq_len > 16) return fail(MDT_ERR_UNSUPPORTED, "action_seq_len must be 1..16");
    const int n_tok = c.arch == MDT_ARCH_MDTV ? c.n_obs_token : 2;
    const int cond = !c.use_ada_conditioning ? COND_TOKEN : (c.use_noise_encoder ? COND_NOISE : COND_ADALN);
    const int sig_tok = cond == COND_TOKEN ? 1 : 0;
    const bool prop = c.use_proprio != 0;
    if (prop && c.arch != MDT_ARCH_MDTV)
        return fail(MDT_ERR_INVALID_ARG, "use_proprio: only MDTVTransformer reads state['state_obs'] "
                                         "(MDTTransformer.process_state_embeddings returns None, mdt_transformer.py:309-316)");
    if (prop && (c.proprio_dim < 1 || c.proprio_dim > 16)) return fail(MDT_ERR_UNSUPPORTED, "proprio_dim must be 1..16");
    if (n_tok < 1 || sig_tok + 1 + n_tok + (prop ? 1 : 0) > 16)
        return fail(MDT_ERR_UNSUPPORTED, "context length must be <= 16 tokens");
    const bool gc = c.no_goal_conditioning == 0;
// ... 305 lines not shown
    if (mr.mod && mr.gate >= 0) { p.mod = mr.mod; p.mod_stride = mr.stride; p.gate_off = mr.gate; }
    if (B <= ATTN_PROJ_MAX_BATCH && mdt_attn_proj_supported(p, m->H, m->hd, T, m->cfg.use_rot_embed)) {
        LAUNCH(mdt_launch_attn_proj(p, V.qkv, 3 * D, m->H, m->hd, T, causal, s));
        return MDT_OK;
    }
    if (fx && fused && M >= g_attn_xattn_min_rows() && B <= ATTN_XATTN_MAX_BATCH &&
        mdt_attn_xattn_supported(p, *fx, m->H, m->hd, T, causal, m->cfg.use_rot_embed)) {
        LAUNCH(mdt_launch_attn_xattn(p, V.qkv, 3 * D, *fx, m->H, m->hd, T, s));
        *fused = true;
        return MDT_OK;
    }
    const int64_t wide_tiles = (int64_t)((M + 31) / 32) * ((D + 127) / 128);
    if (M >= g_attn_wide_min_rows() && (wide_tiles <= 256 || g_attn_wide_override > 0) &&
        mdt_attn_proj_wide_supported(p, m->H, m->hd, T, causal, m->cfg.use_rot_embed)) {
        LAUNCH(mdt_launch_attn_proj_wide(p, V.qkv, 3 * D, m->H, m->hd, T, s));
        return MDT_OK;
    }
    mdt_attn_args a;
    memset(&a, 0, sizeof a);
    a.q = V.qkv; a.ldq = 3 * D; a.k = V.qkv + D; a.v = V.qkv + 2 * D; a.ldkv = 3 * D;
    a.out = V.att; a.ldo = D; a.B = (int)B; a.H = m->H; a.hd = m->hd; a.Tq = T; a.Tk = T;
    a.causal = causal; a.rope = m->cfg.use_rot_embed;
    LAUNCH(mdt_launch_attention(a, m->rope_cos, m->rope_sin, s));
    LAUNCH(mdt_launch_gemm(p, s));
    return MDT_OK;
}

static int g_mlp_fuse_override = -1;
static int g_mlp_fuse_min_rows(bool split = false) {
    if (g_mlp_fuse_override >= 0) return g_mlp_fuse_override == 0 ? 1 << 30 : g_mlp_fuse_override;
    return split ? mdt_split_min_rows() : 1401;
}
extern "C" void mdt_op_set_mlp_fuse_min(int32_t rows) { g_mlp_fuse_override = rows; }

static bool g_trace_mlp = false;
struct TraceEv { hipEvent_t e0, e1, e2; };
static std::vector<TraceEv> g_trace_mlp_events;
static std::vector<float> g_trace_mlp_empty;
extern "C" void mdt_op_trace_mlp(int32_t enable) { g_trace_mlp = enable != 0; }
extern "C" int32_t mdt_op_trace_mlp_read(float* us, int32_t cap) {
    int32_t n = 0;
    g_trace_mlp_empty.clear();
    for (auto& ev : g_trace_mlp_events) {
        float ms = 0.f, ms0 = 0.f;
        if (hipEventSynchronize(ev.e2) == hipSuccess && hipEventElapsedTime(&ms, ev.e0, ev.e1) == hipSuccess &&
            hipEventElapsedTime(&ms0, ev.e1, ev.e2) == hipSuccess && us && n < cap) {
            us[n++] = ms * 1e3f;
            g_trace_mlp_empty.push_back(ms0 * 1e3f);
        }
        (void)hipEventDestroy(ev.e0); (void)hipEventDestroy(ev.e1); (void)hipEventDestroy(ev.e2);
    }
    g_trace_mlp_events.clear();
    return n;
}
extern "C" int32_t mdt_op_trace_mlp_read_empty(float* us, int32_t cap) {
    int32_t n = 0;
    for (float v : g_trace_mlp_empty)
        if (us && n < cap) us[n++] = v;
    return n;
}

__global__ void k_clock_stamp(uint64_t* __restrict__ out) {
    if (threadIdx.x == 0) {
        unsigned xcc;
        asm volatile("s_getreg_b32 %0, hwreg(HW_REG_XCC_ID)" : "=s"(xcc));
        xcc &= 7u;
        out[2 * xcc] = __builtin_amdgcn_s_memtime();
        out[2 * xcc + 1] = __builtin_amdgcn_s_memrealtime();
    }
}
extern "C" mdt_status mdt_op_clock_stamp(uint64_t* out16, void* stream) {
    if (!out16) return fail(MDT_ERR_INVALID_ARG, "mdt_op_clock_stamp: null output");
    hipLaunchKernelGGL(k_clock_stamp, dim3(64), dim3(64), 0, (hipStream_t)stream, out16);
    HIP_TRY(hipGetLastError());
    return MDT_OK;
}

static mdt_status refresh_split(mdt_model* m, hipStream_t s) {
    auto one = [&](const Lin& l) -> mdt_status {
        if (l.ws) LAUNCH(mdt_launch_split_from_packed(l.wp, l.N, l.K, l.ws, s));
        return MDT_OK;
    };
    for (const EncBlock& e : m->enc) { MDT_TRY(one(e.qkv)); MDT_TRY(one(e.fc)); MDT_TRY(one(e.proj2)); }
    for (const DecBlock& d : m->dec) { MDT_TRY(one(d.qkv)); MDT_TRY(one(d.fc)); MDT_TRY(one(d.proj2)); }
    m->split_stale = false;
    return MDT_OK;
}
static inline mdt_status split_ready(mdt_model* m, int64_t rows, hipStream_t s) {
    if (m->split_stale && mdt_mlp_split_enabled() && rows >= mdt_split_min_rows()) return refresh_split(m, s);
    return MDT_OK;
}

static mdt_status run_mlp(mdt_model* m, const EncBlock& e, const View& V, int64_t B, int T, ModRef mr, hipStream_t s,
                          Stream* out = nullptr, const mdt_xapply_args* pre_x = nullptr) {
    float* x = V.y;
    const int D = m->D, M = (int)(B * T);
    mdt_gemm_args g = gemm_args(x, D, e.fc, V.hid, 4 * D, M);
    g.ln = 1; g.ln_w = e.ln2_w; g.ln_b = e.ln2_b; g.act = MDT_ACT_GELU;
    g.rows_per_sample = T;
    if (mr.mod && mr.shift >= 0) { g.mod = mr.mod; g.mod_stride = mr.stride; g.shift_off = mr.shift; g.scale_off = mr.scale; }
    mdt_gemm_args p = gemm_args(V.hid, 4 * D, e.proj2, pre_x ? pre_x->y_out : x, D, M);
    p.residual = 1; p.rows_per_sample = T;
    if (mr.mod && mr.gate >= 0) { p.mod = mr.mod; p.mod_stride = mr.stride; p.gate_off = mr.gate; }
    if (out) *out = Stream();
    const bool split = e.fc.ws && e.proj2.ws && mdt_mlp_split_enabled() && M >= mdt_split_min_rows() && mdt_mlp_split_supported(g, p);
    if (out && !pre_x && M >= g_mlp_fuse_min_rows(split) && mdt_mlp_slices(D) >= 2 && mdt_mlp_supported(g, p)) {
        p.ldo = D;
        const int64_t stride = (int64_t)M * D;
        if (g_trace_mlp) {
            TraceEv ev;
            HIP_TRY(hipEventCreate(&ev.e0)); HIP_TRY(hipEventCreate(&ev.e1)); HIP_TRY(hipEventCreate(&ev.e2));
            HIP_TRY(hipEventRecord(ev.e0, s));
            if (split) LAUNCH(mdt_launch_mlp_split(g, p, e.fc.ws, e.proj2.ws, V.hid, stride, s));
            else LAUNCH(mdt_launch_mlp(g, p, V.hid, stride, s));
            HIP_TRY(hipEventRecord(ev.e1, s));
            HIP_TRY(hipEventRecord(ev.e2, s));
            g_trace_mlp_events.push_back(ev);
        } else if (split) {
            LAUNCH(mdt_launch_mlp_split(g, p, e.fc.ws, e.proj2.ws, V.hid, stride, s));
        } else {
            LAUNCH(mdt_launch_mlp(g, p, V.hid, stride, s));
        }
        out->base = V.hid; out->parts = mdt_mlp_slices(D); out->stride = stride;
        return MDT_OK;
    }
    if (pre_x) LAUNCH(mdt_launch_xattn_gemm(*pre_x, g, s));
    else LAUNCH(mdt_launch_gemm(g, s));
    LAUNCH(mdt_launch_gemm(p, s));
    return MDT_OK;
}

static constexpr int64_t XATTN_FC_MAX_BATCH = 2;

static mdt_status run_sigma_mlp(mdt_model* m, const float* sigma, int64_t sstride, int R, float* out, int64_t ldo,
                                int gout, int act, hipStream_t s, bool emb_done = false, bool side = false) {
    const int D = m->D;
    if (!emb_done) LAUNCH(mdt_launch_sigma_emb(sigma, sstride, m->freqs, m->sig_e, R, D, s));
    mdt_gemm_args a = gemm_args(m->sig_e, D, m->sig1, m->sig_t, 2 * D, R);
    a.act = MDT_ACT_MISH;
    LAUNCH(side ? mdt_gemm_side_push(a, s) : mdt_launch_gemm(a, s));
    mdt_gemm_args b = gemm_args(m->sig_t, 2 * D, m->sig3, out, ldo, R);
    b.act = act;
    b.gin = 1; b.gout = gout; b.goff = 0;
    LAUNCH(side ? mdt_gemm_side_push(b, s) : mdt_launch_gemm(b, s));
    return MDT_OK;
}

static mdt_status check_encode_args(const mdt_model* m, const float* tokens, const float* tokens2, const float* goal,
                                    const float* ctx_out) {
    if (!tokens || !goal) return fail(MDT_ERR_INVALID_ARG, "encode: null tokens/goal");
    if (m->cfg.arch == MDT_ARCH_MDT && !tokens2) return fail(MDT_ERR_INVALID_ARG, "encode: MDT needs the gripper tokens");
    if (m->p_row >= 0 && !tokens2)
        return fail(MDT_ERR_INVALID_ARG, "encode: this handle was created with use_proprio; state_obs (tokens2) is required");
    if (misaligned(tokens) || misaligned(goal) || misaligned(tokens2) || misaligned(ctx_out))
        return fail(MDT_ERR_INVALID_ARG, "encode: pointers must be 16-byte aligned");
    return MDT_OK;
}

static mdt_status run_encode(mdt_model* m, const float* tokens, const float* tokens2, const float* goal, int modality,
                             int honour_modality, int64_t B, const float* sigma, int64_t sstride, float* ctx_out,
                             hipStream_t s) {
    const mdt_config& c = m->cfg;
    const int D = m->D, Te = m->Te;
    const int t0 = m->sig_tok;
    if (t0 && !sigma)
        return fail(MDT_ERR_INVALID_ARG, "encode: use_ada_conditioning=False puts sigma into the context; sigma is required");
    MDT_TRY(check_encode_args(m, tokens, tokens2, goal, ctx_out));
    MDT_TRY(check_loaded(m));
    MDT_TRY(mdt_reserve(m, B));
    MDT_TRY(split_ready(m, B * std::max(m->Te, m->Ta), s));
    m->cached_batch = 0;
    const bool lang = honour_modality && c.use_modality_encoder && modality == MDT_MODALITY_LANG;
    const Lin& g0 = lang ? m->lang0 : m->goal0;
    const Lin& g2 = lang ? m->lang2 : m->goal2;
    const float* pos0 = (c.arch == MDT_ARCH_MDT && c.use_abs_pos_emb) ? m->pos_emb : nullptr;
    const float* pos1 = pos0 ? m->pos_emb + (int64_t)c.goal_seq_len * D : nullptr;
    if (t0) MDT_TRY(run_sigma_mlp(m, sigma, sstride, (int)B, m->h_enc, D, Te, MDT_ACT_NONE, s));
    const bool tok_side = c.arch == MDT_ARCH_MDTV && m->g_row >= 0 && B * m->n_tok <= 15;
    const size_t side_before = mdt_gemm_side_pending();
    if (tok_side) {
        mdt_gemm_args a = gemm_args(tokens, m->O, m->tok, m->h_enc, D, (int)(B * m->n_tok));
        a.gin = m->n_tok; a.gout = Te; a.goff = m->tok_row;
        LAUNCH(mdt_gemm_side_push_front(a, s));
    }
    if (m->g_row >= 0) {
        const float* gin = goal;
        int64_t ld = m->G;
        if (c.use_mlp_goal) {
            mdt_gemm_args a = gemm_args(goal, m->G, g0, m->hid, 2 * D, (int)B);
            a.act = MDT_ACT_GELU;
            LAUNCH(mdt_launch_gemm(a, s));
            gin = m->hid; ld = 2 * D;
        }
        mdt_gemm_args a = gemm_args(gin, ld, g2, m->h_enc, D, (int)B);
        a.gin = 1; a.gout = Te; a.goff = m->g_row; a.rowvec = pos0;
        LAUNCH(mdt_launch_gemm(a, s));
    }
    if (tok_side && mdt_gemm_side_pending() > side_before) LAUNCH(mdt_gemm_side_launch_front(s));
    if (c.arch == MDT_ARCH_MDTV) {
        if (!tok_side) {
            mdt_gemm_args a = gemm_args(tokens, m->O, m->tok, m->h_enc, D, (int)(B * m->n_tok));
            a.gin = m->n_tok; a.gout = Te; a.goff = m->tok_row;
            LAUNCH(mdt_launch_gemm(a, s));
        }
    } else {
        mdt_gemm_args a = gemm_args(tokens, m->O, m->tok, m->h_enc, D, (int)B);
        a.gin = 1; a.gout = Te; a.goff = m->tok_row; a.rowvec = pos1;
        LAUNCH(mdt_launch_gemm(a, s));
        mdt_gemm_args b2 = gemm_args(tokens2, m->O, m->incam, m->h_enc, D, (int)B);
        b2.gin = 1; b2.gout = Te; b2.goff = m->tok_row + 1; b2.rowvec = pos1;
        LAUNCH(mdt_launch_gemm(b2, s));
    }
    if (m->p_row >= 0) {
        LAUNCH(mdt_launch_narrow_linear(tokens2, m->prop0_T, m->prop0_b, nullptr, m->hid, (int)B, m->Pd, 2 * D, MDT_ACT_MISH, s));
        mdt_gemm_args a = gemm_args(m->hid, 2 * D, m->prop2, m->h_enc, D, (int)B);
        a.gin = 1; a.gout = Te; a.goff = m->p_row;
        LAUNCH(mdt_launch_gemm(a, s));
    }
    for (int l = 0; l < m->Le; ++l) {
        MDT_TRY(run_self_attn(m, m->enc[l], encoder_view(m), B, Te, false, ModRef(), s));
        MDT_TRY(run_mlp(m, m->enc[l], encoder_view(m), B, Te, ModRef(), s));
    }
    LAUNCH(mdt_launch_layernorm(m->h_enc, m->enc_ln_w, m->enc_ln_b, m->ctx, (int)(B * Te), D, s, ctx_out));
    {
        mdt_gemm_args a = gemm_args(m->ctx, D, m->kv_all, m->kvx, (int64_t)m->Ld * 2 * D, (int)(B * Te));
        LAUNCH(mdt_launch_gemm(a, s));
    }
    if (m->xfold) {
        const int64_t np = (int64_t)4 * m->H;
        std::vector<mdt_xfold_args> sets(m->Ld);
        for (int l = 0; l < m->Ld; ++l) {
            mdt_xfold_args& f = sets[l];
            memset(&f, 0, sizeof f);
            f.kv = m->kvx + (int64_t)l * 2 * D; f.ldkv = (int64_t)m->Ld * 2 * D;
            f.WqT_p = m->dec[l].xq_pT; f.bq = m->dec[l].xq.bias; f.Wo_p = m->dec[l].xproj.wp;
            f.U = m->xU + (int64_t)l * m->cap * np * D; f.Wf = m->xW + (int64_t)l * m->cap * np * D;
            f.c = m->xc + (int64_t)l * m->cap * np;
            f.B = (int)B; f.H = m->H; f.hd = m->hd; f.D = D; f.Te = Te;
        }
        LAUNCH(mdt_launch_xattn_fold_n(sets.data(), m->Ld, s));
    }
    m->cached_batch = B;
    return MDT_OK;
}

static mdt_status run_modulation(mdt_model* m, const float* sigma, int64_t sstride, int R, hipStream_t s, bool emb_done = false,
                                 bool side = false) {
    const int D = m->D;
    if (m->cond == COND_TOKEN) return MDT_OK;
    if (m->cond == COND_NOISE) return run_sigma_mlp(m, sigma, sstride, R, m->cmod, 2 * D, 1, MDT_ACT_NONE, s, emb_done, side);
    MDT_TRY(run_sigma_mlp(m, sigma, sstride, R, m->sig_c, D, 1, MDT_ACT_SILU, s, emb_done, side));
    mdt_gemm_args c = gemm_args(m->sig_c, D, m->mod_all, m->mod, (int64_t)m->Ld * 6 * D, R);
    LAUNCH(side ? mdt_gemm_side_push(c, s) : mdt_launch_gemm(c, s));
    return MDT_OK;
}

static const float* cond_row(const mdt_model* m, int64_t r) {
    if (m->cond == COND_ADALN) return m->mod + r * (int64_t)m->Ld * 6 * m->D;
    if (m->cond == COND_NOISE) return m->cmod + r * 2 * (int64_t)m->D;
    return nullptr;
}
static int64_t cond_width(const mdt_model* m) {
    return m->cond == COND_ADALN ? (int64_t)m->Ld * 6 * m->D : (m->cond == COND_NOISE ? 2 * (int64_t)m->D : 0);
}

static mdt_status run_decoder_blocks(mdt_model* m, const View& V, int64_t B, const float* mod_row, int64_t mod_stride,
                                     hipStream_t s, Stream* fin = nullptr) {
    const int D = m->D, Ta = m->Ta, M = (int)(B * Ta);
    View W = V;
    Stream cur;
    if (fin) *fin = Stream();
    MDT_TRY(split_ready(m, M, s));
    for (int l = 0; l < m->Ld; ++l) {
        const DecBlock& d = m->dec[l];
        ModRef ma, mx, mm;
        if (m->cond == COND_ADALN) {
            const float* row = mod_row + (int64_t)l * 6 * D;
            ma = ModRef(row, mod_stride, 0, D, 2 * D);
            mm = ModRef(row, mod_stride, 3 * D, 4 * D, 5 * D);
        } else if (m->cond == COND_NOISE) {
            ma = mx = ModRef(mod_row, mod_stride, 0, D, -1);
        }
        mdt_xapply_args x;
        memset(&x, 0, sizeof x);
        if (m->xfold) {
            const int64_t np = (int64_t)4 * m->H;
            x.y = W.y; x.ln_w = d.ln3_w; x.ln_b = d.ln3_b; x.bo = d.xproj.bias;
            x.U = m->xU + ((int64_t)l * m->cap + V.b0) * np * D;
            x.Wf = m->xW + ((int64_t)l * m->cap + V.b0) * np * D;
            x.c = m->xc + ((int64_t)l * m->cap + V.b0) * np;
            x.B = (int)B; x.H = m->H; x.D = D; x.Te = m->Te; x.Ta = Ta;
        }
        bool x_in_fc = false;
        if (m->xfold) {
            mdt_gemm_args gf = gemm_args(W.y, D, d.fc, W.hid, 4 * D, M);
            gf.ln = 1; gf.rows_per_sample = Ta;
            x.y_out = W.att;
            x_in_fc = B <= XATTN_FC_MAX_BATCH && M <= 192 && m->Ld % 2 == 0 && mdt_xattn_gemm_supported(x, gf);
            if (!x_in_fc) x.y_out = nullptr;
        }
        bool xdone = false;
        MDT_TRY(run_self_attn(m, d, W, B, Ta, true, ma, s, cur, m->xfold ? &x : nullptr, &xdone));
        cur = Stream();
        if (xdone) {
        } else if (m->xfold) {
            if (!x_in_fc) LAUNCH(mdt_launch_xattn_apply(x, s));
        } else {
            mdt_gemm_args q = gemm_args(W.y, D, d.xq, W.qx, D, M);
// ... 406 lines not shown
extern "C" double mdt_flops_per_chunk(const mdt_model* m, int32_t n_steps) {
    if (!m) return 0.0;
    const double D = m->D, Te = m->Te, Ta = m->Ta, A = m->A, G = m->G, O = m->O;
    auto attn = [&](double Tq, double Tk) { return 2.0 * (2.0 * Tq * Tk * D); };
    double goal = m->g_row < 0 ? 0.0 : (m->cfg.use_mlp_goal ? 2.0 * (G * 2 * D + 2 * D * D) : 2.0 * G * D);
    double enc = goal + 2.0 * m->n_tok * O * D +
                 m->Le * (Te * 2.0 * (4 * D * D + 8 * D * D) + attn(Te, Te));
    double kv = m->Ld * Te * 2.0 * 2 * D * D;
    double sig = 2.0 * (D * 2 * D + 2 * D * D);
    double blk = (m->cond == COND_ADALN ? 2.0 * D * 6 * D : 0.0) + Ta * 2.0 * (4 * D * D) + Ta * 2.0 * (2 * D * D) +
                 Ta * 2.0 * 8 * D * D + attn(Ta, Ta) + attn(Ta, Te);
    const double head = m->HP ? 2.0 * Ta * ((double)D * m->HH + (double)m->HH * A) : 2.0 * Ta * A * D;
    double step = sig + 2.0 * Ta * A * D + head + m->Ld * blk;
    if (m->cond == COND_TOKEN) return n_steps * (enc + kv + step);
    return enc + kv + n_steps * step;
}

extern "C" int64_t mdt_op_packed_numel(int64_t N, int64_t K) { return N * K; }

extern "C" mdt_status mdt_op_pack_weight(const float* w, int64_t n_rows, int64_t K, float* packed, int64_t n_off,
                                         int64_t N_total, void* stream) {
    if (!w || !packed || K % 16 || N_total % 16 || n_off < 0 || n_off + n_rows > N_total)
        return fail(MDT_ERR_INVALID_ARG, "mdt_op_pack_weight: bad argument (N, K must be multiples of 16)");
    LAUNCH(mdt_launch_pack_weight(w, (int)n_rows, (int)K, packed, (int)n_off, (hipStream_t)stream));
    return MDT_OK;
}

extern "C" mdt_status mdt_op_pack_weight_glu(const float* w, int64_t H2, int64_t K, float* packed, void* stream) {
    if (!w || !packed || H2 < 32 || (H2 % 32) || K < 16 || (K % 16) || misaligned(w) || misaligned(packed))
        return fail(MDT_ERR_INVALID_ARG, "mdt_op_pack_weight_glu: (2H, K) with H and K multiples of 16, 16-byte aligned pointers");
    LAUNCH(mdt_launch_pack_weight_glu(w, (int)(H2 / 2), (int)K, packed, (hipStream_t)stream));
    return MDT_OK;
}

extern "C" mdt_status mdt_op_gemm(const mdt_gemm_args* a, void* stream) {
    if (!a || !a->A || !a->Wp || !a->out) return fail(MDT_ERR_INVALID_ARG, "mdt_op_gemm: null pointer");
    if (a->N % 16 || a->K % 16 || a->lda % 4 || a->ldo % 4 || a->M < 1)
        return fail(MDT_ERR_INVALID_ARG, "mdt_op_gemm: N, K multiples of 16 and lda, ldo multiples of 4 required");
    if (a->ln && a->K > 512) return fail(MDT_ERR_UNSUPPORTED, "mdt_op_gemm: LayerNorm prologue needs K <= 512");
    if (a->gin < 1 || a->rows_per_sample < 1) return fail(MDT_ERR_INVALID_ARG, "mdt_op_gemm: gin/rows_per_sample < 1");
    if (misaligned(a->A) || misaligned(a->Wp) || misaligned(a->out) || misaligned(a->bias) || misaligned(a->mod))
        return fail(MDT_ERR_INVALID_ARG, "mdt_op_gemm: pointers must be 16-byte aligned");
    LAUNCH(mdt_launch_gemm(*a, (hipStream_t)stream));
    return MDT_OK;
}

extern "C" mdt_status mdt_op_mlp(const mdt_gemm_args* fc, const mdt_gemm_args* proj, float* parts, int64_t part_stride,
                                 int32_t* n_parts, void* stream) {
    if (!fc || !proj || !fc->A || !fc->Wp || !proj->Wp || !parts || !fc->ln_w)
        return fail(MDT_ERR_INVALID_ARG, "mdt_op_mlp: null pointer");
    if (!mdt_mlp_supported(*fc, *proj))
        return fail(MDT_ERR_UNSUPPORTED, "mdt_op_mlp: needs D = fc.K a multiple of 128 (<= 512), fc.N = proj.K = 4 D, proj.N = D, "
                                         "a LayerNorm prologue and plain output rows");
    if (fc->lda % 4 || proj->ldo % 4 || proj->ldo < proj->N || part_stride < (int64_t)fc->M * proj->ldo)
        return fail(MDT_ERR_INVALID_ARG, "mdt_op_mlp: lda / ldo multiples of 4, part_stride >= M * ldo required");
    if (misaligned(fc->A) || misaligned(fc->Wp) || misaligned(proj->Wp) || misaligned(parts) || misaligned(fc->bias) ||
        misaligned(proj->bias) || misaligned(fc->mod) || misaligned(proj->mod) || (part_stride & 3))
        return fail(MDT_ERR_INVALID_ARG, "mdt_op_mlp: pointers must be 16-byte aligned");
    LAUNCH(mdt_launch_mlp(*fc, *proj, parts, part_stride, (hipStream_t)stream));
    if (n_parts) *n_parts = mdt_mlp_slices(fc->K);
    return MDT_OK;
}

extern "C" mdt_status mdt_op_pack_weight_split(const float* w, int64_t n_rows, int64_t K, void* image, void* stream) {
    if (!w || !image) return fail(MDT_ERR_INVALID_ARG, "mdt_op_pack_weight_split: null pointer");
    if (n_rows < 16 || n_rows % 16 || K < 32 || K % 32 || n_rows * K >= ((int64_t)1 << 30))
        return fail(MDT_ERR_INVALID_ARG, "mdt_op_pack_weight_split: n_rows a multiple of 16, K a multiple of 32");
    if (misaligned(w) || misaligned(image)) return fail(MDT_ERR_INVALID_ARG, "mdt_op_pack_weight_split: pointers must be 16-byte aligned");
    LAUNCH(mdt_launch_pack_weight_split(w, (int)n_rows, (int)K, image, (hipStream_t)stream));
    return MDT_OK;
}

extern "C" mdt_status mdt_op_pack_weight_split_rows(const float* w, int64_t n_rows, int64_t K, void* image, int64_t n_off, void* stream) {
    if (!w || !image) return fail(MDT_ERR_INVALID_ARG, "mdt_op_pack_weight_split_rows: null pointer");
    if (n_rows < 1 || n_off < 0 || n_off % 16 || K < 32 || K % 32 || (n_rows + n_off) * K >= ((int64_t)1 << 30))
        return fail(MDT_ERR_INVALID_ARG, "mdt_op_pack_weight_split_rows: n_off a multiple of 16, K a multiple of 32");
    if (misaligned(w) || misaligned(image)) return fail(MDT_ERR_INVALID_ARG, "mdt_op_pack_weight_split_rows: pointers must be 16-byte aligned");
    LAUNCH(mdt_launch_pack_weight_split(w, (int)n_rows, (int)K, image, (hipStream_t)stream, (int)n_off));
    return MDT_OK;
}

extern "C" mdt_status mdt_op_mlp_split(const mdt_gemm_args* fc, const mdt_gemm_args* proj, const void* fc_split, const void* proj_split,
                                       float* parts, int64_t part_stride, int32_t* n_parts, void* stream) {
    if (!fc || !proj || !fc->A || !fc_split || !proj_split || !parts || !fc->ln_w)
        return fail(MDT_ERR_INVALID_ARG, "mdt_op_mlp_split: null pointer");
    if (!mdt_mlp_split_supported(*fc, *proj))
        return fail(MDT_ERR_UNSUPPORTED, "mdt_op_mlp_split: needs D = fc.K a multiple of 128 (<= 512), fc.N = proj.K = 4 D, proj.N = D, "
                                         "a LayerNorm prologue and plain output rows");
    if (fc->lda % 4 || proj->ldo % 4 || proj->ldo < proj->N || part_stride < (int64_t)fc->M * proj->ldo)
        return fail(MDT_ERR_INVALID_ARG, "mdt_op_mlp_split: lda / ldo multiples of 4, part_stride >= M * ldo required");
    if (misaligned(fc->A) || misaligned(fc_split) || misaligned(proj_split) || misaligned(parts) || misaligned(fc->bias) ||
        misaligned(proj->bias) || misaligned(fc->mod) || misaligned(proj->mod) || (part_stride & 3))
        return fail(MDT_ERR_INVALID_ARG, "mdt_op_mlp_split: pointers must be 16-byte aligned");
    LAUNCH(mdt_launch_mlp_split(*fc, *proj, fc_split, proj_split, parts, part_stride, (hipStream_t)stream));
    if (n_parts) *n_parts = mdt_mlp_slices(fc->K);
    return MDT_OK;
}

extern "C" mdt_status mdt_op_attention(const mdt_attn_args* a, void* stream) {
    if (!a || !a->q || !a->k || !a->v || !a->out) return fail(MDT_ERR_INVALID_ARG, "mdt_op_attention: null pointer");
    if (a->Tq < 1 || a->Tq > 16 || a->Tk < 1 || a->Tk > 16) return fail(MDT_ERR_UNSUPPORTED, "Tq, Tk must be 1..16");
    if (a->hd != 16 && a->hd != 32 && a->hd != 48 && a->hd != 64) return fail(MDT_ERR_UNSUPPORTED, "hd must be 16/32/48/64");
    if (a->rope) {
        if (a->hd < 32) return fail(MDT_ERR_INVALID_ARG, "rope needs hd >= 32");
        static float *cs = nullptr, *sn = nullptr;
        if (!cs) {
            std::vector<float> rc(256), rs(256);
            for (int i = 0; i < 16; ++i) {
                const float f = 1.0f / powf(10000.0f, (float)(2 * i) / 32.0f);
                for (int p = 0; p < 16; ++p) { rc[p * 16 + i] = cosf((float)p * f); rs[p * 16 + i] = sinf((float)p * f); }
            }
            HIP_TRY(hipMalloc((void**)&cs, 256 * sizeof(float)));
            HIP_TRY(hipMalloc((void**)&sn, 256 * sizeof(float)));
            HIP_TRY(hipMemcpy(cs, rc.data(), 256 * sizeof(float), hipMemcpyHostToDevice));
            HIP_TRY(hipMemcpy(sn, rs.data(), 256 * sizeof(float), hipMemcpyHostToDevice));
        }
        LAUNCH(mdt_launch_attention(*a, cs, sn, (hipStream_t)stream));
        return MDT_OK;
    }
    LAUNCH(mdt_launch_attention(*a, nullptr, nullptr, (hipStream_t)stream));
    return MDT_OK;
}

extern "C" mdt_status mdt_op_xattn_fold(const mdt_xfold_args* a, void* stream) {
    if (!a || !a->kv || !a->WqT_p || !a->bq || !a->Wo_p || !a->U || !a->Wf || !a->c)
        return fail(MDT_ERR_INVALID_ARG, "mdt_op_xattn_fold: null pointer");
    if (a->H * a->hd != a->D || a->Te < 1 || a->Te > 4 || a->D > 512 || a->D % 128 || (a->H != 4 && a->H != 8) || a->hd % 16)
        return fail(MDT_ERR_UNSUPPORTED, "mdt_op_xattn_fold: need 4 or 8 heads of 16 / 32 / 48 / 64, H*hd == D <= 512 a multiple of 128 "
                                         "and 1 <= Te <= 4");
    if (misaligned(a->U) || misaligned(a->Wf) || misaligned(a->c) || misaligned(a->kv) || (a->ldkv & 3))
        return fail(MDT_ERR_INVALID_ARG, "mdt_op_xattn_fold: kv / U / Wf / c must be 16-byte aligned, ldkv a multiple of 4");
    LAUNCH(mdt_launch_xattn_fold(*a, (hipStream_t)stream));
    return MDT_OK;
}

extern "C" mdt_status mdt_op_xattn_apply(const mdt_xapply_args* a, void* stream) {
    if (!a || !a->y || !a->ln_w || !a->U || !a->Wf || !a->c) return fail(MDT_ERR_INVALID_ARG, "mdt_op_xattn_apply: null pointer");
    if (!mdt_xattn_apply_supported(a->D, a->H, a->Te, a->Ta))
        return fail(MDT_ERR_UNSUPPORTED, "mdt_op_xattn_apply: unsupported (D, H, Te, Ta) = (%d, %d, %d, %d): needs 4 or 8 heads, D <= 512 a "
                                         "multiple of 128, 1 <= Te <= 4, Ta <= 16", a->D, a->H, a->Te, a->Ta);
    if (misaligned(a->y) || misaligned(a->y_out) || misaligned(a->U) || misaligned(a->Wf) || misaligned(a->c) || misaligned(a->ln_w) ||
        misaligned(a->ln_b) || misaligned(a->bo))
        return fail(MDT_ERR_INVALID_ARG, "mdt_op_xattn_apply: pointers must be 16-byte aligned");
    LAUNCH(mdt_launch_xattn_apply(*a, (hipStream_t)stream));
    return MDT_OK;
}

extern "C" mdt_status mdt_op_attn_proj(const mdt_gemm_args* proj, const float* qkv, int64_t ldq, int32_t hd, int32_t T,
                                       int32_t causal, void* stream) {
    if (!proj || !qkv || !proj->Wp || !proj->out) return fail(MDT_ERR_INVALID_ARG, "mdt_op_attn_proj: null argument");
    if (T >= 1 && proj->M / T > 64 && mdt_attn_proj_wide_supported(*proj, 8, hd, T, causal, 0)) {
        if (misaligned(qkv) || misaligned(proj->Wp) || misaligned(proj->out) || (ldq & 3))
            return fail(MDT_ERR_INVALID_ARG, "mdt_op_attn_proj: pointers must be 16-byte aligned, ldq a multiple of 4");
        LAUNCH(mdt_launch_attn_proj_wide(*proj, qkv, ldq, 8, hd, T, (hipStream_t)stream));
        return MDT_OK;
    }
    if (!mdt_attn_proj_supported(*proj, 8, hd, T, 0))
        return fail(MDT_ERR_UNSUPPORTED, "mdt_op_attn_proj: needs 8 heads of 16/32/48/64 (K = 8 * hd), T <= 16 rows per sample "
                                         "(M = samples * T, at most 64 samples), a plain projection");
    LAUNCH(mdt_launch_attn_proj(*proj, qkv, ldq, 8, hd, T, causal, (hipStream_t)stream));
    return MDT_OK;
}

extern "C" mdt_status mdt_op_xattn_gemm(const mdt_xapply_args* x, const mdt_gemm_args* g, void* stream) {
    if (!x || !g || !x->y || !x->ln_w || !x->U || !x->Wf || !x->c || !g->Wp || !g->out || !g->ln_w)
        return fail(MDT_ERR_INVALID_ARG, "mdt_op_xattn_gemm: null argument");
    if (misaligned(x->y) || misaligned(x->y_out) || misaligned(x->U) || misaligned(x->Wf) || misaligned(x->c) || misaligned(g->Wp) ||
        misaligned(g->out))
        return fail(MDT_ERR_INVALID_ARG, "mdt_op_xattn_gemm: pointers must be 16-byte aligned");
    if (!mdt_xattn_gemm_supported(*x, *g))
        return fail(MDT_ERR_UNSUPPORTED, "mdt_op_xattn_gemm: needs a cross-attention mdt_op_xattn_apply supports with its own output array "
                                         "(y_out != y) and a LayerNorm-prologue Linear on the same rows (A == x->y, lda = K = D, M = B * Ta, "
                                         "rows_per_sample = Ta, N a multiple of 16, no residual / row remap)");
    LAUNCH(mdt_launch_xattn_gemm(*x, *g, (hipStream_t)stream));
    return MDT_OK;
}

extern "C" mdt_status mdt_op_attn_xattn(const mdt_gemm_args* proj, const float* qkv, int64_t ldq, const mdt_xapply_args* x,
// ... 36 lines not shown
```

### mdt_policy_amd/csrc/mdt_tiles.h

```cpp
#pragma once
#include <hip/hip_runtime.h>
#include <stdint.h>

#include "mdt_internal.h"
#include "mdt_device.h"

__device__ __forceinline__ int xcd_remap(int bid, int nblocks) {
    const int q = nblocks >> 3, r = nblocks & 7, xcd = bid & 7, idx = bid >> 3;
    return (xcd < r ? xcd * (q + 1) : r * (q + 1) + (xcd - r) * q) + idx;
}

typedef unsigned u32x4_t __attribute__((ext_vector_type(4)));
template <bool COH>
struct ActLd;
template <>
struct ActLd<false> {
    const float* base;
    __device__ __forceinline__ explicit ActLd(const float* p) : base(p) {}
    __device__ __forceinline__ f32x4 ld4(int64_t off) const { return ldg4(base + off); }
    __device__ __forceinline__ float ld1(int64_t off) const { return base[off]; }
};
template <>
struct ActLd<true> {
    __amdgpu_buffer_rsrc_t rsrc;
// ... 15 lines not shown
};
__device__ __forceinline__ WStream wstream(const float* image, int64_t float_off) {
    return WStream{__builtin_amdgcn_make_buffer_rsrc((void*)image, 0, 0xffffffffu, 0x00020000), (unsigned)(float_off << 2)};
}
__device__ __forceinline__ f32x4 wld4(const WStream& w) {
    return __builtin_bit_cast(f32x4, __builtin_amdgcn_raw_buffer_load_b128(w.rs, w.off, 0, 0));
}

enum { PRO_PLAIN = 0, PRO_LN = 1, PRO_LN_MOD_BCAST = 2, PRO_LN_MOD_ROWS = 3,
       PRO_ATTN = 4  };

struct mdt_attn_pro {
    const float* qkv;
    int64_t ldq;
    int T;
    float scale;
};

__device__ __forceinline__ void st4(float* p, f32x4 v) {
    asm volatile("global_store_dwordx4 %0, %1, off sc0 sc1\n\ts_nop 1" ::"v"(p), "v"(v) : "memory");
}
__device__ __forceinline__ f32x4 sel4(bool c, f32x4 a, f32x4 b) { return c ? a : b; }
__device__ __forceinline__ float hsum4(f32x4 v) { return (v.x + v.y) + (v.z + v.w); }
__device__ __forceinline__ float hsq4(f32x4 v) { return (v.x * v.x + v.y * v.y) + (v.z * v.z + v.w * v.w); }

#if defined(MDT_DEBUG_TIMING) && defined(MDT_TILES_TIMING_OWNER)
__device__ unsigned long long* g_dbg_ts = nullptr;
#define MDT_TS(i)                                                                         \
    if (threadIdx.x == 0 && g_dbg_ts != nullptr) {                                        \
        g_dbg_ts[(size_t)blockIdx.x * 8 + (i)] = __builtin_readcyclecounter();            \
    }
#define MDT_TS2(i)                                                                        \
    if ((threadIdx.x & 255) == 0 && g_dbg_ts != nullptr) {                               \
        g_dbg_ts[((size_t)blockIdx.x + (threadIdx.x >> 8) * gridDim.x) * 8 + (i)] = __builtin_readcyclecounter(); \
    }
#define MDT_TSO(off, i)                                                                   \
    if (threadIdx.x == 0 && g_dbg_ts != nullptr) {                                        \
        g_dbg_ts[((size_t)blockIdx.x + (off)) * 8 + (i)] = __builtin_readcyclecounter();  \
    }
#define MDT_TS_HWID()                                                                     \
    if (threadIdx.x == 0 && g_dbg_ts != nullptr) {                                        \
        unsigned hw, xcc;                                                                 \
        asm volatile("s_getreg_b32 %0, hwreg(HW_REG_HW_ID)" : "=s"(hw));                  \
        asm volatile("s_getreg_b32 %0, hwreg(HW_REG_XCC_ID)" : "=s"(xcc));                \
        g_dbg_ts[(size_t)blockIdx.x * 8 + 7] = ((unsigned long long)xcc << 32) | hw;      \
    }
#else
#define MDT_TS(i)
#define MDT_TS2(i)
#define MDT_TSO(off, i)
#define MDT_TS_HWID()
#endif

#define MDT_PRIO(x) if constexpr (KSTEP_PRIO) __builtin_amdgcn_s_setprio(x);
#define MDT_SCHED_PIN __builtin_amdgcn_sched_barrier(0x6);
#define MDT_KSTEP(U, KC)                                                                                  \
    {                                                                                                     \
        const int kpf = min(kg + (KC) + R - 1, K16 - 1);                                                  \
        _Pragma("unroll") for (int j = 0; j < NTW; ++j) ring[((U) + R - 1) % R][j] = wld4(wp[j] + kpf * 256); \
        MDT_SCHED_PIN                                                                                     \
        MDT_PRIO(1)                                                                                       \
        MDT_KSTEP_MFMAS(U, 0)                                                                             \
        MDT_SCHED_PIN                                                                                     \
        f32x4 avn[MTILES];  \
        _Pragma("unroll") for (int i = 0; i < MTILES; ++i) avn[i] =                                       \
            *(const f32x4*)(ap + i * 16 * stride + min((KC) + 1, nk - 1) * 16);                           \
        MDT_SCHED_PIN                                                                                     \
        MDT_KSTEP_MFMAS(U, 1)                                                                             \
        MDT_KSTEP_MFMAS(U, 2)                                                                             \
        MDT_KSTEP_MFMAS(U, 3)                                                                             \
        MDT_PRIO(0)                                                                                       \
        MDT_SCHED_PIN                                                                                     \
        _Pragma("unroll") for (int i = 0; i < MTILES; ++i) av[i] = avn[i];                                \
    }
#define MDT_KSTEP_MFMAS(U, E)                                                                             \
    _Pragma("unroll") for (int i = 0; i < MTILES; ++i) {                                                  \
        _Pragma("unroll") for (int j = 0; j < NTW; ++j) acc[i][j] =                                       \
            __builtin_amdgcn_mfma_f32_16x16x4f32(ring[(U)][j][(E)], av[i][(E)], acc[i][j], 0, 0, 0);      \
    }

template <int MTILES, int NWAVES, int PRO, bool COH, int XP = 1, int XB = 2, bool SPLIT = false>
__device__ __forceinline__ void gemm_stage_tile(const mdt_gemm_args& a, float* lds, int stride, int m0, int k0, int klen,
                                                const float* __restrict__ zeros, int tid, int lane, int wave,
                                                float* merge_out = nullptr) {
    static_assert(!SPLIT || PRO != PRO_PLAIN, "the split store belongs to the LayerNorm prologues");
    constexpr int MT = MTILES * 16;
    constexpr int NT = 64 * NWAVES;
    const f32x4 zero4 = (f32x4){0.f, 0.f, 0.f, 0.f};
    const int n4 = klen >> 2;
    const ActLd<COH> LA(a.A);
    if constexpr (PRO != PRO_PLAIN) {
        constexpr int RPW = MT / NWAVES;
        const int r0 = wave * RPW;
        int cc[2];
        bool cv[2];
#pragma unroll
        for (int p = 0; p < 2; ++p) {
            cv[p] = lane + 64 * p < n4;
            cc[p] = 4 * min(lane + 64 * p, n4 - 1);
        }
        f32x4 v[RPW][2], w[2], bb[2];
#pragma unroll
        for (int r = 0; r < RPW; ++r) {
            const int64_t m = min(m0 + r0 + r, a.M - 1);
#pragma unroll
            for (int p = 0; p < 2; ++p) v[r][p] = LA.ld4(m * a.lda + cc[p]);
        }
        if constexpr (XP > 1) {
            constexpr int HB = XB == 1 || RPW < 2 ? RPW : RPW / 2;
#pragma unroll
            for (int r0b = 0; r0b < RPW; r0b += HB) {
                f32x4 vx[XP - 1][HB][2];
#pragma unroll
                for (int x = 1; x < XP; ++x)
#pragma unroll
                    for (int r = 0; r < HB; ++r) {
                        const int64_t m = min(m0 + r0 + r0b + r, a.M - 1);
#pragma unroll
                        for (int p = 0; p < 2; ++p) vx[x - 1][r][p] = LA.ld4((int64_t)x * a.a_part_stride + m * a.lda + cc[p]);
                    }
#pragma unroll
                for (int r = 0; r < HB; ++r)
#pragma unroll
                    for (int p = 0; p < 2; ++p) {
#pragma unroll
                        for (int x = 1; x < XP; ++x) v[r0b + r][p] = v[r0b + r][p] + vx[x - 1][r][p];
                        if (merge_out != nullptr && cv[p] && m0 + r0 + r0b + r < a.M)
                            st4(merge_out + (int64_t)(m0 + r0 + r0b + r) * a.lda + cc[p], v[r0b + r][p]);
                    }
            }
        }
        const float* lnb = a.ln_b != nullptr ? a.ln_b : zeros;
#pragma unroll
        for (int p = 0; p < 2; ++p) {
            w[p] = ldg4(a.ln_w + cc[p]);
            bb[p] = ldg4(lnb + cc[p]);
        }
        constexpr int NC = PRO == PRO_LN_MOD_ROWS ? 2 : 1;
        f32x4 sh[NC][2], sc[NC][2];
        int s_lo = 0;
        bool slow_mod = false;
        if constexpr (PRO == PRO_LN_MOD_BCAST) {
#pragma unroll
            for (int p = 0; p < 2; ++p) {
                sh[0][p] = ldg4(a.mod + a.shift_off + cc[p]);
                sc[0][p] = ldg4(a.mod + a.scale_off + cc[p]);
            }
        }
        if constexpr (PRO == PRO_LN_MOD_ROWS) {
            s_lo = min(m0 + r0, a.M - 1) / a.rows_per_sample;
            const int s_hi = min(m0 + r0 + RPW - 1, a.M - 1) / a.rows_per_sample;
            slow_mod = s_hi > s_lo + 1;
            const float* mlo = a.mod + (int64_t)s_lo * a.mod_stride;
            const float* mhi = a.mod + (int64_t)min(s_lo + 1, s_hi) * a.mod_stride;
#pragma unroll
            for (int p = 0; p < 2; ++p) {
                sh[0][p] = ldg4(mlo + a.shift_off + cc[p]);
                sc[0][p] = ldg4(mlo + a.scale_off + cc[p]);
                sh[NC - 1][p] = ldg4(mhi + a.shift_off + cc[p]);
                sc[NC - 1][p] = ldg4(mhi + a.scale_off + cc[p]);
            }
        }
        const float inv_k = 1.0f / (float)klen;
        float red[RPW];
#pragma unroll
        for (int r = 0; r < RPW; ++r) {
            red[r] = 0.f;
#pragma unroll
            for (int p = 0; p < 2; ++p) {
                v[r][p] = sel4(cv[p], v[r][p], zero4);
                red[r] += hsum4(v[r][p]);
            }
        }
        wave_sum_n<RPW>(red);
#pragma unroll
        for (int r = 0; r < RPW; ++r) {
            const float mean = red[r] * inv_k;
            red[r] = 0.f;
#pragma unroll
            for (int p = 0; p < 2; ++p) {
                v[r][p] = sel4(cv[p], v[r][p] - mean, zero4);
                red[r] += hsq4(v[r][p]);
            }
        }
        wave_sum_n<RPW>(red);
#pragma unroll
        for (int r = 0; r < RPW; ++r) {
            const int m = m0 + r0 + r;
            const float rstd = 1.0f / sqrtf(red[r] * inv_k + 1e-5f);
#pragma unroll
            for (int p = 0; p < 2; ++p) {
                f32x4 y = v[r][p] * rstd * w[p] + bb[p];
                if constexpr (PRO == PRO_LN_MOD_BCAST) y = sh[0][p] + y * sc[0][p];
                if constexpr (PRO == PRO_LN_MOD_ROWS) {
                    const int smp = min(m, a.M - 1) / a.rows_per_sample;
                    f32x4 shv = sel4(smp == s_lo, sh[0][p], sh[NC - 1][p]);
                    f32x4 scv = sel4(smp == s_lo, sc[0][p], sc[NC - 1][p]);
                    if (slow_mod) {
                        const float* mr = a.mod + (int64_t)smp * a.mod_stride;
                        shv = ldg4(mr + a.shift_off + cc[p]);
                        scv = ldg4(mr + a.scale_off + cc[p]);
                    }
                    y = shv + y * scv;
                }
                y = sel4(m < a.M, y, zero4);
                if constexpr (SPLIT) {
                    if (cv[p]) {
                        mdt_bf16x4 p1, p2, p3;
                        split3_bf16(y, p1, p2, p3);
                        char* q = (char*)lds + split_slot(r0 + r, cc[p], stride);
                        *(mdt_bf16x4*)q = p1;
                        *(mdt_bf16x4*)(q + MT * stride) = p2;
                        *(mdt_bf16x4*)(q + 2 * MT * stride) = p3;
                    }
                } else {
                    if (cv[p]) *(f32x4*)(lds + (r0 + r) * stride + cc[p]) = y;
                }
            }
        }
    } else {
        constexpr int RG = NT / 32;
        constexpr int U = MT / RG;
        const int rg = tid >> 5, l32 = tid & 31;
        const int nv = (n4 + 31) >> 5;
        for (int v0 = 0; v0 < nv; v0 += 3) {
            f32x4 st[U][3];
#pragma unroll
            for (int u = 0; u < U; ++u) {
                const int64_t m = min(m0 + rg + RG * u, a.M - 1);
#pragma unroll
                for (int v = 0; v < 3; ++v)
                    st[u][v] = LA.ld4(m * a.lda + k0 + 4 * min(l32 + 32 * (v0 + v), n4 - 1));
            }
#pragma unroll
            for (int u = 0; u < U; ++u) {
                const int row = rg + RG * u;
#pragma unroll
                for (int v = 0; v < 3; ++v) {
                    const int c4 = l32 + 32 * (v0 + v);
                    if (c4 < n4) *(f32x4*)(lds + row * stride + 4 * c4) = sel4(m0 + row < a.M, st[u][v], zero4);
                }
            }
        }
    }
}

__device__ __forceinline__ float quad_sum(float v) {
    v += dpp_get<0xB1, 0xf>(v);
    v += dpp_get<0x4E, 0xf>(v);
    return v;
}
template <int HD, int TKC>
__device__ __forceinline__ void attn_stage_tile(const mdt_gemm_args& a, const mdt_attn_pro& ap, float* xa, int stride, int m0,
                                                float* scratch, int tid) {
    constexpr int HH = 4, HHD = HH * HD, ST = HHD + 16, H4 = HHD / 4, KVR = 48, DS = HD / 4, NL = 12;
    const f32x4 zero4 = (f32x4){0.f, 0.f, 0.f, 0.f};
    const int T = ap.T, D = 2 * HHD;
    const int kv0 = (m0 / T) * T;
    const int nkv = min(m0 + 32, a.M) - kv0;
    float* qs = scratch;
    float* ks = qs + 32 * ST;
    float* vs = ks + KVR * ST;
    const int nq4 = 32 * H4, nk4 = nkv * H4, total = nq4 + 2 * nk4;
    f32x4 t[2][NL];
#pragma unroll
    for (int hh = 0; hh < 2; ++hh)
#pragma unroll
        for (int u = 0; u < NL; ++u) {
            const int idx = min(tid + 512 * u, total - 1);
            int64_t src;
            if (idx < nq4) {
                const int r = idx / H4, c = idx - r * H4;
                src = (int64_t)min(m0 + r, a.M - 1) * ap.ldq + hh * HHD + 4 * c;
            } else {
                const int i2 = idx - nq4, which = i2 >= nk4, i3 = i2 - which * nk4, r = i3 / H4, c = i3 - r * H4;
                src = (int64_t)(kv0 + r) * ap.ldq + (1 + which) * D + hh * HHD + 4 * c;
            }
            t[hh][u] = ldg4(ap.qkv + src);
        }
    const int lp = tid & 3, pr = tid >> 2, r = pr & 31, hl = pr >> 5;
    const int m = m0 + r;
    const bool valid = m < a.M;
    const int mc = min(m, a.M - 1), smp = mc / T, tq = mc - smp * T;
    const int kb = smp * T - kv0;
    const int d0 = hl * HD + lp * DS;
#pragma unroll
    for (int hh = 0; hh < 2; ++hh) {
        if (hh) __syncthreads();
// ... 1323 lines not shown
```

Before: 76680.

## Fuse encoder final LayerNorm into split KV GEMM and add narrow MLP slices

```diff
diff --git a/include/mdt_hip_ops.h b/include/mdt_hip_ops.h
--- a/include/mdt_hip_ops.h
+++ b/include/mdt_hip_ops.h
@@ -56,6 +56,9 @@
 mdt_status mdt_op_pack_weight_split_rows(const float *w, int64_t n_rows, int64_t K, void *image, int64_t n_off, void *stream);
 mdt_status mdt_op_mlp_split(const mdt_gemm_args *fc, const mdt_gemm_args *proj, const void *fc_split, const void *proj_split,
                             float *parts, int64_t part_stride, int32_t *n_parts, void *stream);
+mdt_status mdt_op_mlp_split_slice(const mdt_gemm_args *fc, const mdt_gemm_args *proj, const void *fc_split, const void *proj_split,
+                                  float *parts, int64_t part_stride, int32_t hidden_slice, int32_t *n_parts, void *stream);
+mdt_status mdt_op_gemm_ln_out(const mdt_gemm_args *args, float *ln_out, float *ln_out2, void *stream);
 void mdt_op_set_mlp_split(int32_t on);
 void mdt_op_set_mlp_fuse_min(int32_t rows);
 void mdt_op_set_side_jobs(int32_t on);
diff --git a/mdt_policy_amd/_lib.py b/mdt_policy_amd/_lib.py
--- a/mdt_policy_amd/_lib.py
+++ b/mdt_policy_amd/_lib.py
@@ -225,6 +225,8 @@
     ("mdt_op_pack_weight_split", _I32, [_VP, _I64, _I64, _VP, _VP]),
     ("mdt_op_pack_weight_split_rows", _I32, [_VP, _I64, _I64, _VP, _I64, _VP]),
     ("mdt_op_mlp_split", _I32, [C.POINTER(GemmArgs), C.POINTER(GemmArgs), _VP, _VP, _VP, _I64, C.POINTER(_I32), _VP]),
+    ("mdt_op_mlp_split_slice", _I32, [C.POINTER(GemmArgs), C.POINTER(GemmArgs), _VP, _VP, _VP, _I64, _I32, C.POINTER(_I32), _VP]),
+    ("mdt_op_gemm_ln_out", _I32, [C.POINTER(GemmArgs), _VP, _VP, _VP]),
     ("mdt_op_set_mlp_split", None, [_I32]),
     ("mdt_op_set_gemm_geometry", None, [_I32]),
     ("mdt_op_set_mlp_fuse_min", None, [_I32]),
diff --git a/mdt_policy_amd/csrc/mdt_internal.h b/mdt_policy_amd/csrc/mdt_internal.h
--- a/mdt_policy_amd/csrc/mdt_internal.h
+++ b/mdt_policy_amd/csrc/mdt_internal.h
@@ -70,7 +70,10 @@
 bool mdt_mlp_split_enabled();
 int mdt_split_min_rows();
 hipError_t mdt_launch_mlp_split(const mdt_gemm_args& fc, const mdt_gemm_args& proj, const void* w1s, const void* w2s, float* parts,
-                                int64_t part_stride, hipStream_t s);
+                                int64_t part_stride, hipStream_t s, int hidden_slice = 512);
+int mdt_mlp_split_hidden_slice(const mdt_gemm_args& fc);
+bool mdt_gemm_ln_split_applies(const mdt_gemm_args& a);
+hipError_t mdt_launch_gemm_ln_out(const mdt_gemm_args& a, float* ln_out, float* ln_out2, hipStream_t s);
 hipError_t mdt_launch_pack_weight_split(const float* w, int n_rows, int K, void* image, hipStream_t s, int n_off = 0);
 hipError_t mdt_launch_split_from_packed(const float* wp, int N, int K, void* image, hipStream_t s);
 hipError_t mdt_launch_attention(const mdt_attn_args& a, const float* rope_cos, const float* rope_sin, hipStream_t s);
diff --git a/mdt_policy_amd/csrc/mdt_kernels.hip b/mdt_policy_amd/csrc/mdt_kernels.hip
--- a/mdt_policy_amd/csrc/mdt_kernels.hip
+++ b/mdt_policy_amd/csrc/mdt_kernels.hip
@@ -188,7 +188,7 @@
     mlp_tile<NTW2, PRO>(f, p, parts, part_stride, by, s, lds, zeros, threadIdx.x, skew);
 }
 
-template <int NTW2, int PRO>
+template <int NTW2, int PRO, int HS = 512>
 __global__ __launch_bounds__(512) void k_mlp_split(mdt_gemm_args f, mdt_gemm_args p, const char* __restrict__ w1s, const char* __restrict__ w2s,
                                                    float* __restrict__ parts, int64_t part_stride, int n_slices, int gm,
                                                    const float* __restrict__ zeros) {
@@ -197,7 +197,7 @@
     const int i = blockIdx.x >> 3, w = (blockIdx.x & 7) * per + i;
     if (i >= per || w >= total) return;
     const int s = w / gm, by = w - s * gm;
-    mlp_split_tile<NTW2, PRO>(f, p, w1s, w2s, parts, part_stride, by, s, lds_c, zeros, threadIdx.x);
+    mlp_split_tile<NTW2, PRO, HS>(f, p, w1s, w2s, parts, part_stride, by, s, lds_c, zeros, threadIdx.x);
 }
 
 template <int MTILES, int NTW, int NWAVES, int LW, bool RES>
@@ -682,7 +682,7 @@
 
 static hipError_t launch_gemm_merge(const mdt_gemm_args& a, hipStream_t s);
 static bool gemm_ln_split_applies(const mdt_gemm_args& a);
-static hipError_t launch_gemm_ln_split(const mdt_gemm_args& a, hipStream_t s);
+static hipError_t launch_gemm_ln_split(const mdt_gemm_args& a, hipStream_t s, float* ln_out = nullptr, float* ln_out2 = nullptr);
 
 bool mdt_attn_proj_wide_supported(const mdt_gemm_args& p, int H, int hd, int T, int causal, int rope) {
     return w_image_ok(p.N, p.K) && H == 8 && (hd == 16 || hd == 32 || hd == 48) && p.K == H * hd && T >= 1 && T <= 16 && causal && !rope && p.residual &&
@@ -936,14 +936,15 @@
 }
 
 template <int ND, int NTW, int PRO, int XP>
-__global__ __launch_bounds__(512) void k_gemm_ln_split(mdt_gemm_args a, int grid_n, const float* __restrict__ zeros) {
+__global__ __launch_bounds__(512) void k_gemm_ln_split(mdt_gemm_args a, int grid_n, const float* __restrict__ zeros, float* ln_out,
+                                                       float* ln_out2) {
     extern __shared__ __attribute__((aligned(16))) char lds_c[];
     const int logical = xcd_remap(blockIdx.x, gridDim.x);
     const int by = logical / grid_n, bx = logical - by * grid_n;
-    gemm_ln_split_tile<ND, NTW, PRO, XP>(a, by, bx, lds_c, zeros, threadIdx.x);
+    gemm_ln_split_tile<ND, NTW, PRO, XP>(a, by, bx, lds_c, zeros, threadIdx.x, ln_out, ln_out2);
 }
 template <int ND, int NTW, int PRO, int XP>
-static hipError_t launch_gemm_ln_split_t(const mdt_gemm_args& a, hipStream_t s) {
+static hipError_t launch_gemm_ln_split_t(const mdt_gemm_args& a, float* ln_out, float* ln_out2, hipStream_t s) {
     const int gn = a.N / (8 * NTW * 16), gm = (a.M + 31) / 32;
     const int lds = 3 * 32 * (2 * 128 * ND + 32);
     static bool attr_dev[MAX_DEVICES] = {false};
@@ -953,31 +954,46 @@
         if (e != hipSuccess) return e;
         done = true;
     }
-    hipLaunchKernelGGL((k_gemm_ln_split<ND, NTW, PRO, XP>), dim3(gn * gm), dim3(512), lds, s, a, gn, g_zeros);
+    hipLaunchKernelGGL((k_gemm_ln_split<ND, NTW, PRO, XP>), dim3(gn * gm), dim3(512), lds, s, a, gn, g_zeros, ln_out, ln_out2);
     return hipGetLastError();
 }
 template <int ND, int NTW, int PRO>
-static hipError_t launch_gemm_ln_split_x(const mdt_gemm_args& a, hipStream_t s) {
+static hipError_t launch_gemm_ln_split_x(const mdt_gemm_args& a, float* ln_out, float* ln_out2, hipStream_t s) {
     switch (a.a_parts) {
-        case 2: return launch_gemm_ln_split_t<ND, NTW, PRO, 2>(a, s);
-        case 3: return launch_gemm_ln_split_t<ND, NTW, PRO, 3>(a, s);
-        case 4: return launch_gemm_ln_split_t<ND, NTW, PRO, 4>(a, s);
-        default: return launch_gemm_ln_split_t<ND, NTW, PRO, 1>(a, s);
+        case 2: return launch_gemm_ln_split_t<ND, NTW, PRO, 2>(a, ln_out, ln_out2, s);
+        case 3: return launch_gemm_ln_split_t<ND, NTW, PRO, 3>(a, ln_out, ln_out2, s);
+        case 4: return launch_gemm_ln_split_t<ND, NTW, PRO, 4>(a, ln_out, ln_out2, s);
+        case 6:
+            if constexpr (ND == 3 && PRO == PRO_LN) return launch_gemm_ln_split_t<ND, NTW, PRO, 6>(a, ln_out, ln_out2, s);
+            return hipErrorInvalidValue;
+        default: return launch_gemm_ln_split_t<ND, NTW, PRO, 1>(a, ln_out, ln_out2, s);
     }
 }
 template <int ND, int NTW>
-static hipError_t launch_gemm_ln_split_pro(const mdt_gemm_args& a, hipStream_t s) {
+static hipError_t launch_gemm_ln_split_pro(const mdt_gemm_args& a, float* ln_out, float* ln_out2, hipStream_t s) {
     if (a.mod != nullptr && a.shift_off >= 0)
-        return a.mod_stride == 0 ? launch_gemm_ln_split_x<ND, NTW, PRO_LN_MOD_BCAST>(a, s) : launch_gemm_ln_split_x<ND, NTW, PRO_LN_MOD_ROWS>(a, s);
-    return launch_gemm_ln_split_x<ND, NTW, PRO_LN>(a, s);
+        return a.mod_stride == 0 ? launch_gemm_ln_split_x<ND, NTW, PRO_LN_MOD_BCAST>(a, ln_out, ln_out2, s)
+                                 : launch_gemm_ln_split_x<ND, NTW, PRO_LN_MOD_ROWS>(a, ln_out, ln_out2, s);
+    return launch_gemm_ln_split_x<ND, NTW, PRO_LN>(a, ln_out, ln_out2, s);
 }
 static bool gemm_ln_split_applies(const mdt_gemm_args& a) {
+    const bool parts_ok = a.a_parts <= 4 || (a.a_parts == 6 && a.K == 384 && (a.mod == nullptr || a.shift_off < 0));
     return a.Wp_split != nullptr && mdt_mlp_split_enabled() && a.ln && (a.K == 384 || a.K == 512) && a.N % 384 == 0 &&
            a.M >= mdt_split_min_rows() && a.batch <= 1 && !a.residual && a.gin == 1 && a.gout == 1 && a.goff == 0 && a.rowvec == nullptr && !a.aux_mode &&
-           a.a_parts <= 4 && (a.lda & 3) == 0 && (a.ldo & 3) == 0 && g_mdt_gemm_force == 0;
-}
-static hipError_t launch_gemm_ln_split(const mdt_gemm_args& a, hipStream_t s) {
-    return a.K == 512 ? launch_gemm_ln_split_pro<4, 3>(a, s) : launch_gemm_ln_split_pro<3, 3>(a, s);
+           parts_ok && (a.lda & 3) == 0 && (a.ldo & 3) == 0 && g_mdt_gemm_force == 0;
+}
+bool mdt_gemm_ln_split_applies(const mdt_gemm_args& a) { return gemm_ln_split_applies(a); }
+static bool gemm_ln_split_narrow(const mdt_gemm_args& a) { return (int64_t)((a.M + 31) / 32) * (a.N / 384) < 128; }
+static hipError_t launch_gemm_ln_split(const mdt_gemm_args& a, hipStream_t s, float* ln_out, float* ln_out2) {
+    const bool narrow = gemm_ln_split_narrow(a);
+    if (a.K == 512) return narrow ? launch_gemm_ln_split_pro<4, 1>(a, ln_out, ln_out2, s) : launch_gemm_ln_split_pro<4, 3>(a, ln_out, ln_out2, s);
+    return narrow ? launch_gemm_ln_split_pro<3, 1>(a, ln_out, ln_out2, s) : launch_gemm_ln_split_pro<3, 3>(a, ln_out, ln_out2, s);
+}
+hipError_t mdt_launch_gemm_ln_out(const mdt_gemm_args& a, float* ln_out, float* ln_out2, hipStream_t s) {
+    if (!gemm_ln_split_applies(a) || ln_out == nullptr) return hipErrorInvalidValue;
+    hipError_t ze = ensure_zeros();
+    if (ze != hipSuccess) return ze;
+    return launch_gemm_ln_split(a, s, ln_out, ln_out2);
 }
 
 static int g_mlp_split = -1;
@@ -990,20 +1006,20 @@
 bool mdt_mlp_split_supported(const mdt_gemm_args& f, const mdt_gemm_args& p) {
     return mdt_mlp_supported(f, p);
 }
-template <int NTW2, int PRO>
+template <int NTW2, int PRO, int HS = 512>
 static hipError_t launch_mlp_split_t(const mdt_gemm_args& f, const mdt_gemm_args& p, const void* w1s, const void* w2s, float* parts,
                                      int64_t part_stride, hipStream_t s) {
-    const int S = mdt_mlp_slices(f.K), gm = (f.M + 31) / 32;
-    const int lds = mlp_split_lds_bytes(128 * NTW2);
+    const int S = 4 * f.K / HS, gm = (f.M + 31) / 32;
+    const int lds = mlp_split_lds_bytes(128 * NTW2, HS);
     static bool attr_dev[MAX_DEVICES] = {false};
     bool& done = attr_dev[current_device()];
     if (!done) {
-        hipError_t e = hipFuncSetAttribute((const void*)k_mlp_split<NTW2, PRO>, hipFuncAttributeMaxDynamicSharedMemorySize, lds);
+        hipError_t e = hipFuncSetAttribute((const void*)k_mlp_split<NTW2, PRO, HS>, hipFuncAttributeMaxDynamicSharedMemorySize, lds);
         if (e != hipSuccess) return e;
         done = true;
     }
     const int per = (gm * S + 7) / 8;
-    hipLaunchKernelGGL((k_mlp_split<NTW2, PRO>), dim3(8 * per), dim3(512), lds, s, f, p, (const char*)w1s, (const char*)w2s, parts,
+    hipLaunchKernelGGL((k_mlp_split<NTW2, PRO, HS>), dim3(8 * per), dim3(512), lds, s, f, p, (const char*)w1s, (const char*)w2s, parts,
                        part_stride, S, gm, g_zeros);
     return hipGetLastError();
 }
@@ -1015,11 +1031,24 @@
                                  : launch_mlp_split_t<NTW2, PRO_LN_MOD_ROWS>(f, p, w1s, w2s, parts, part_stride, s);
     return launch_mlp_split_t<NTW2, PRO_LN>(f, p, w1s, w2s, parts, part_stride, s);
 }
+int mdt_mlp_split_hidden_slice(const mdt_gemm_args& f) {
+    const bool plain = f.mod == nullptr || f.shift_off < 0;
+    return plain && (f.K == 256 || f.K == 384) && (int64_t)((f.M + 31) / 32) * (4 * f.K / 512) < 128 ? 256 : 512;
+}
 hipError_t mdt_launch_mlp_split(const mdt_gemm_args& f, const mdt_gemm_args& p, const void* w1s, const void* w2s, float* parts,
-                                int64_t part_stride, hipStream_t s) {
+                                int64_t part_stride, hipStream_t s, int hidden_slice) {
     if (!mdt_mlp_split_supported(f, p) || !w1s || !w2s) return hipErrorInvalidValue;
+    if (hidden_slice != 512 && hidden_slice != 256) return hipErrorInvalidValue;
     hipError_t ze = ensure_zeros();
     if (ze != hipSuccess) return ze;
+    if (hidden_slice == 256) {
+        if (f.mod != nullptr && f.shift_off >= 0) return hipErrorInvalidValue;
+        switch (f.K / 128) {
+            case 2: return launch_mlp_split_t<2, PRO_LN, 256>(f, p, w1s, w2s, parts, part_stride, s);
+            case 3: return launch_mlp_split_t<3, PRO_LN, 256>(f, p, w1s, w2s, parts, part_stride, s);
+            default: return hipErrorInvalidValue;
+        }
+    }
     switch (f.K / 128) {
         case 1: return launch_mlp_split_pro<1>(f, p, w1s, w2s, parts, part_stride, s);
         case 2: return launch_mlp_split_pro<2>(f, p, w1s, w2s, parts, part_stride, s);
diff --git a/mdt_policy_amd/csrc/mdt_mlp_split.h b/mdt_policy_amd/csrc/mdt_mlp_split.h
--- a/mdt_policy_amd/csrc/mdt_mlp_split.h
+++ b/mdt_policy_amd/csrc/mdt_mlp_split.h
@@ -85,16 +85,17 @@
     }
 }
 
-__host__ __device__ constexpr int mlp_split_lds_bytes(int D) {
-    const int xs = 3 * 32 * (2 * D + 32), hs = 3 * 32 * (2 * 512 + 32);
+__host__ __device__ constexpr int mlp_split_lds_bytes(int D, int HS = 512) {
+    const int xs = 3 * 32 * (2 * D + 32), hs = 3 * 32 * (2 * HS + 32);
     return xs > hs ? xs : hs;
 }
 
-template <int NTW2, int PRO>
+template <int NTW2, int PRO, int HS = 512>
 __device__ __forceinline__ void mlp_split_tile(const mdt_gemm_args& f, const mdt_gemm_args& p, const char* __restrict__ w1s,
                                                const char* __restrict__ w2s, float* __restrict__ parts, int64_t part_stride, int by,
                                                int s, char* lds, const float* __restrict__ zeros, int tid) {
-    constexpr int MTILES = 2, NWAVES = 8, MT = 32, HS = 512, NTW1 = 4, R = 2;
+    static_assert(HS == 512 || HS == 256, "hidden slice of 512 or 256 columns");
+    constexpr int MTILES = 2, NWAVES = 8, MT = 32, NTW1 = HS / 128, R = 2;
     constexpr int D = 128 * NTW2, K32a = D / 32, K32b = HS / 32;
     constexpr int ROWB1 = 2 * D + 32, PART1 = MT * ROWB1, ROWB2 = 2 * HS + 32, PART2 = MT * ROWB2;
     static_assert(NTW2 >= 1 && NTW2 <= 4, "D <= 512");
@@ -190,7 +191,8 @@
 }
 
 template <int ND, int NTW, int PRO, int XP>
-__device__ __forceinline__ void gemm_ln_split_tile(const mdt_gemm_args& a, int by, int bx, char* lds, const float* __restrict__ zeros, int tid) {
+__device__ __forceinline__ void gemm_ln_split_tile(const mdt_gemm_args& a, int by, int bx, char* lds, const float* __restrict__ zeros, int tid,
+                                                   float* ln_out = nullptr, float* ln_out2 = nullptr) {
     constexpr int MTILES = 2, NWAVES = 8, MT = 32, R = 2;
     constexpr int D = 128 * ND, K32 = D / 32, ROWB = 2 * D + 32, PART = MT * ROWB;
     static_assert(ND >= 1 && ND <= 4, "D <= 512");
@@ -210,7 +212,8 @@
         for (int j = 0; j < NTW; ++j) bias_v[j] = ldg4(bp + (nt0 + j) * 16 + nq);
     }
     gemm_stage_tile<MTILES, NWAVES, PRO, false, XP, (NTW <= 3 && XP <= 3) ? 1 : 2, true>(a, (float*)xs, ROWB, m0, 0, D, zeros, tid, lane, wave,
-                                                                                         bx == 0 ? a.a_merged : nullptr);
+                                                                                         bx == 0 ? a.a_merged : nullptr,
+                                                                                         bx == 0 ? ln_out : nullptr, bx == 0 ? ln_out2 : nullptr);
     __syncthreads();
     f32x4 acc[MTILES][NTW];
 #pragma unroll
diff --git a/mdt_policy_amd/csrc/mdt_model.hip b/mdt_policy_amd/csrc/mdt_model.hip
--- a/mdt_policy_amd/csrc/mdt_model.hip
+++ b/mdt_policy_amd/csrc/mdt_model.hip
@@ -225,17 +225,21 @@
     if (xb) raw(m->enc_ln_b, P + "encoder.ln.bias", D);
 
     lin_begin(m->kv_all, m->Ld * 2 * D, D, true);
+    const bool kv_split = D % 128 == 0 && D <= 512;
+    if (kv_split) m->kv_all.ws = b.take((size_t)m->Ld * 2 * D * D * 6 / 4);
     if (m->cond == COND_ADALN) lin_begin(m->mod_all, m->Ld * 6 * D, D, true);
     for (int l = 0; l < m->Ld; ++l) {
         const std::string pre = P + "decoder.blocks." + std::to_string(l);
         DecBlock& d = m->dec[l];
         block_common_a(d, pre);
         lin_part(m->kv_all, pre + ".cross_att.key", D, l * 2 * D, true);
+        if (kv_split) add_extra(pre + ".cross_att.key.weight", (int64_t)D * D, SLOT_PACK_SPLIT, (float*)m->kv_all.ws, D, D, l * 2 * D);
         lin_begin(d.xq, D, D, true);
         lin_part(d.xq, pre + ".cross_att.query", D, 0, true);
         d.xq_pT = b.take((size_t)D * D);
         add_extra(pre + ".cross_att.query.weight", (int64_t)D * D, SLOT_PACK_T, d.xq_pT, D, D);
         lin_part(m->kv_all, pre + ".cross_att.value", D, l * 2 * D + D, true);
+        if (kv_split) add_extra(pre + ".cross_att.value.weight", (int64_t)D * D, SLOT_PACK_SPLIT, (float*)m->kv_all.ws, D, D, l * 2 * D + D);
         lin_begin(d.xproj, D, D, xb);
         lin_part(d.xproj, pre + ".cross_att.c_proj", D, 0, xb);
         raw(d.ln3_w, pre + ".ln3.weight", D);
@@ -707,6 +711,7 @@
         return MDT_OK;
     };
     for (const EncBlock& e : m->enc) { MDT_TRY(one(e.qkv)); MDT_TRY(one(e.fc)); MDT_TRY(one(e.proj2)); }
+    MDT_TRY(one(m->kv_all));
     for (const DecBlock& d : m->dec) { MDT_TRY(one(d.qkv)); MDT_TRY(one(d.fc)); MDT_TRY(one(d.proj2)); }
     m->split_stale = false;
     return MDT_OK;
@@ -717,7 +722,7 @@
 }
 
 static mdt_status run_mlp(mdt_model* m, const EncBlock& e, const View& V, int64_t B, int T, ModRef mr, hipStream_t s,
-                          Stream* out = nullptr, const mdt_xapply_args* pre_x = nullptr) {
+                          Stream* out = nullptr, const mdt_xapply_args* pre_x = nullptr, bool narrow_ok = false) {
     float* x = V.y;
     const int D = m->D, M = (int)(B * T);
     mdt_gemm_args g = gemm_args(x, D, e.fc, V.hid, 4 * D, M);
@@ -732,21 +737,25 @@
     if (out && !pre_x && M >= g_mlp_fuse_min_rows(split) && mdt_mlp_slices(D) >= 2 && mdt_mlp_supported(g, p)) {
         p.ldo = D;
         const int64_t stride = (int64_t)M * D;
+        int hs = 512;
+        if (split && narrow_ok && mdt_mlp_split_hidden_slice(g) == 256 &&
+            (int64_t)(4 * D / 256) * M <= (int64_t)4 * m->cap * std::max(m->Te, m->Ta))
+            hs = 256;
         if (g_trace_mlp) {
             TraceEv ev;
             HIP_TRY(hipEventCreate(&ev.e0)); HIP_TRY(hipEventCreate(&ev.e1)); HIP_TRY(hipEventCreate(&ev.e2));
             HIP_TRY(hipEventRecord(ev.e0, s));
-            if (split) LAUNCH(mdt_launch_mlp_split(g, p, e.fc.ws, e.proj2.ws, V.hid, stride, s));
+            if (split) LAUNCH(mdt_launch_mlp_split(g, p, e.fc.ws, e.proj2.ws, V.hid, stride, s, hs));
             else LAUNCH(mdt_launch_mlp(g, p, V.hid, stride, s));
             HIP_TRY(hipEventRecord(ev.e1, s));
             HIP_TRY(hipEventRecord(ev.e2, s));
             g_trace_mlp_events.push_back(ev);
         } else if (split) {
-            LAUNCH(mdt_launch_mlp_split(g, p, e.fc.ws, e.proj2.ws, V.hid, stride, s));
+            LAUNCH(mdt_launch_mlp_split(g, p, e.fc.ws, e.proj2.ws, V.hid, stride, s, hs));
         } else {
             LAUNCH(mdt_launch_mlp(g, p, V.hid, stride, s));
         }
-        out->base = V.hid; out->parts = mdt_mlp_slices(D); out->stride = stride;
+        out->base = V.hid; out->parts = 4 * D / hs; out->stride = stride;
         return MDT_OK;
     }
     if (pre_x) LAUNCH(mdt_launch_xattn_gemm(*pre_x, g, s));
@@ -842,13 +851,33 @@
         a.gin = 1; a.gout = Te; a.goff = m->p_row;
         LAUNCH(mdt_launch_gemm(a, s));
     }
+    const View EV = encoder_view(m);
+    const int Me = (int)(B * Te);
+    mdt_gemm_args kv = gemm_args(m->h_enc, D, m->kv_all, m->kvx, (int64_t)m->Ld * 2 * D, Me);
+    kv.ln = 1; kv.ln_w = m->enc_ln_w; kv.ln_b = m->enc_ln_b;
+    const bool kv_split = mdt_gemm_ln_split_applies(kv);
+    auto takes_six = [&](mdt_gemm_args a) { a.a_parts = 6; return mdt_gemm_ln_split_applies(a); };
+    Stream cur;
     for (int l = 0; l < m->Le; ++l) {
-        MDT_TRY(run_self_attn(m, m->enc[l], encoder_view(m), B, Te, false, ModRef(), s));
-        MDT_TRY(run_mlp(m, m->enc[l], encoder_view(m), B, Te, ModRef(), s));
-    }
-    LAUNCH(mdt_launch_layernorm(m->h_enc, m->enc_ln_w, m->enc_ln_b, m->ctx, (int)(B * Te), D, s, ctx_out));
-    {
-        mdt_gemm_args a = gemm_args(m->ctx, D, m->kv_all, m->kvx, (int64_t)m->Ld * 2 * D, (int)(B * Te));
+        const EncBlock& e = m->enc[l];
+        const bool last = l == m->Le - 1;
+        MDT_TRY(run_self_attn(m, e, EV, B, Te, false, ModRef(), s, cur));
+        cur = Stream();
+        const bool leave = e.fc.ws && e.proj2.ws && mdt_mlp_split_enabled() && Me >= mdt_split_min_rows() && (!last || kv_split);
+        bool narrow_ok = false;
+        if (leave) {
+            mdt_gemm_args q = gemm_args(EV.y, D, last ? m->kv_all : m->enc[l + 1].qkv, EV.qkv, last ? kv.N : 3 * D, Me);
+            q.ln = 1; q.ln_w = last ? m->enc_ln_w : m->enc[l + 1].ln1_w;
+            narrow_ok = takes_six(q);
+        }
+        MDT_TRY(run_mlp(m, e, EV, B, Te, ModRef(), s, leave ? &cur : nullptr, nullptr, narrow_ok));
+    }
+    if (kv_split) {
+        if (cur.parts > 1) { kv.A = cur.base; kv.a_parts = cur.parts; kv.a_part_stride = cur.stride; kv.a_merged = m->h_enc; }
+        LAUNCH(mdt_launch_gemm_ln_out(kv, m->ctx, ctx_out, s));
+    } else {
+        LAUNCH(mdt_launch_layernorm(m->h_enc, m->enc_ln_w, m->enc_ln_b, m->ctx, Me, D, s, ctx_out));
+        mdt_gemm_args a = gemm_args(m->ctx, D, m->kv_all, m->kvx, (int64_t)m->Ld * 2 * D, Me);
         LAUNCH(mdt_launch_gemm(a, s));
     }
     if (m->xfold) {
@@ -1421,6 +1450,11 @@
 
 extern "C" mdt_status mdt_op_mlp_split(const mdt_gemm_args* fc, const mdt_gemm_args* proj, const void* fc_split, const void* proj_split,
                                        float* parts, int64_t part_stride, int32_t* n_parts, void* stream) {
+    return mdt_op_mlp_split_slice(fc, proj, fc_split, proj_split, parts, part_stride, 512, n_parts, stream);
+}
+
+extern "C" mdt_status mdt_op_mlp_split_slice(const mdt_gemm_args* fc, const mdt_gemm_args* proj, const void* fc_split, const void* proj_split,
+                                             float* parts, int64_t part_stride, int32_t hidden_slice, int32_t* n_parts, void* stream) {
     if (!fc || !proj || !fc->A || !fc_split || !proj_split || !parts || !fc->ln_w)
         return fail(MDT_ERR_INVALID_ARG, "mdt_op_mlp_split: null pointer");
     if (!mdt_mlp_split_supported(*fc, *proj))
@@ -1431,8 +1465,22 @@
     if (misaligned(fc->A) || misaligned(fc_split) || misaligned(proj_split) || misaligned(parts) || misaligned(fc->bias) ||
         misaligned(proj->bias) || misaligned(fc->mod) || misaligned(proj->mod) || (part_stride & 3))
         return fail(MDT_ERR_INVALID_ARG, "mdt_op_mlp_split: pointers must be 16-byte aligned");
-    LAUNCH(mdt_launch_mlp_split(*fc, *proj, fc_split, proj_split, parts, part_stride, (hipStream_t)stream));
-    if (n_parts) *n_parts = mdt_mlp_slices(fc->K);
+    if (hidden_slice != 512 && !(hidden_slice == 256 && (fc->K == 256 || fc->K == 384) && (!fc->mod || fc->shift_off < 0)))
+        return fail(MDT_ERR_UNSUPPORTED, "mdt_op_mlp_split: hidden_slice 512, or 256 with D = 256 / 384 and no modulation");
+    LAUNCH(mdt_launch_mlp_split(*fc, *proj, fc_split, proj_split, parts, part_stride, (hipStream_t)stream, hidden_slice));
+    if (n_parts) *n_parts = 4 * fc->K / hidden_slice;
+    return MDT_OK;
+}
+
+extern "C" mdt_status mdt_op_gemm_ln_out(const mdt_gemm_args* a, float* ln_out, float* ln_out2, void* stream) {
+    if (!a || !a->A || !a->Wp_split || !a->out || !a->ln_w || !ln_out) return fail(MDT_ERR_INVALID_ARG, "mdt_op_gemm_ln_out: null pointer");
+    if (misaligned(a->A) || misaligned(a->Wp_split) || misaligned(a->out) || misaligned(a->bias) || misaligned(a->a_merged) ||
+        misaligned(ln_out) || misaligned(ln_out2) || (a->a_parts > 1 && (a->a_part_stride & 3)))
+        return fail(MDT_ERR_INVALID_ARG, "mdt_op_gemm_ln_out: pointers must be 16-byte aligned");
+    if (!mdt_gemm_ln_split_applies(*a))
+        return fail(MDT_ERR_UNSUPPORTED, "mdt_op_gemm_ln_out: needs the split LayerNorm-prologue product (K = 384 / 512, N %% 384 == 0, "
+                                         ">= 768 rows, plain output rows, 1..4 slabs or 6 at K = 384 unmodulated)");
+    LAUNCH(mdt_launch_gemm_ln_out(*a, ln_out, ln_out2, (hipStream_t)stream));
     return MDT_OK;
 }
 
diff --git a/mdt_policy_amd/csrc/mdt_tiles.h b/mdt_policy_amd/csrc/mdt_tiles.h
--- a/mdt_policy_amd/csrc/mdt_tiles.h
+++ b/mdt_policy_amd/csrc/mdt_tiles.h
@@ -121,7 +121,7 @@
 template <int MTILES, int NWAVES, int PRO, bool COH, int XP = 1, int XB = 2, bool SPLIT = false>
 __device__ __forceinline__ void gemm_stage_tile(const mdt_gemm_args& a, float* lds, int stride, int m0, int k0, int klen,
                                                 const float* __restrict__ zeros, int tid, int lane, int wave,
-                                                float* merge_out = nullptr) {
+                                                float* merge_out = nullptr, float* ln_out = nullptr, float* ln_out2 = nullptr) {
     static_assert(!SPLIT || PRO != PRO_PLAIN, "the split store belongs to the LayerNorm prologues");
     constexpr int MT = MTILES * 16;
     constexpr int NT = 64 * NWAVES;
@@ -243,6 +243,10 @@
                     y = shv + y * scv;
                 }
                 y = sel4(m < a.M, y, zero4);
+                if (ln_out != nullptr && cv[p] && m < a.M) {
+                    st4(ln_out + (int64_t)m * klen + cc[p], y);
+                    if (ln_out2 != nullptr) st4(ln_out2 + (int64_t)m * klen + cc[p], y);
+                }
                 if constexpr (SPLIT) {
                     if (cv[p]) {
                         mdt_bf16x4 p1, p2, p3;
```

Result: faster. 77680, median of 6 (+1.3%).
